# buaacyw/MeshAnything

Hardware: NVIDIA H100
Metric: face-tokens/sec (350M, 800-face cap) (higher is better)
Workload: dtype f16 weights/activations, f32 accumulate

## Files before the change

include/meshanything_b200.h:

```cpp
#ifndef MESHANYTHING_B200_H
#define MESHANYTHING_B200_H

#include <stddef.h>
#include <stdint.h>

#ifdef __cplusplus
extern "C" {
#endif

#define MA_ABI_VERSION 1
#define MA_MAX_LAYERS 32

#define MA_EPI_NONE 0
#define MA_EPI_RELU 1
#define MA_EPI_GELU 2
#define MA_LIN_SEG64 0x10
#define MA_LIN_SEG256 0x20

int ma_abi_version(void);
const char* ma_last_error(void);


int ma_linear_f16(const void* W, const void* bias, const void* x, int ldx, void* y, int ldy, int M, int N, int K,
                  int epilogue, void* stream);

int ma_layernorm(const float* x, const void* res16, const float* gamma, const float* beta, float eps, int M, int W,
                 float* out32, void* out16, void* stream);

size_t ma_attention_scratch_bytes(int M, int H, int max_keys);
int ma_attention_f16(const void* q, int ldq, const void* K, const void* V, long T, int H, const int* slots,
                     const int* nkeys, int max_keys, int M, float scale, void* out, int ldo, void* scratch,
                     void* stream);
int ma_attention_decode_f16(const void* qkv, int ldq, void* K, void* V, long T, const int* nkeys, int max_keys, int M,
                            float scale, void* out, int ldo, void* scratch, void* stream);


typedef struct {
  int n_layers, vocab, codebook, npos;
  const void* wqkv[MA_MAX_LAYERS];
  const void* bqkv[MA_MAX_LAYERS];
  const void* wo[MA_MAX_LAYERS];
  const void* bo[MA_MAX_LAYERS];
  const void* w1[MA_MAX_LAYERS];
  const void* b1[MA_MAX_LAYERS];
  const void* w2[MA_MAX_LAYERS];
  const void* b2[MA_MAX_LAYERS];
  const float* ln1g[MA_MAX_LAYERS];
  const float* ln1b[MA_MAX_LAYERS];
  const float* ln2g[MA_MAX_LAYERS];
  const float* ln2b[MA_MAX_LAYERS];
  const void* lm_head;
  const void* tok_table;
  const float* extra;
  const float* tok_pos;
  const float* cond;
  const float* pos;
} ma_decoder_weights;

typedef struct {
  int do_sample;
  int top_k;
  float top_p;
  uint64_t seed;
} ma_sampling;

int ma_sample_tokens(const void* logits, int B, int vocab, const ma_sampling* sampling, int32_t* out_tokens,
                     int32_t* out_support, void* stream);

size_t ma_kv_cache_bytes(int n_layers, int B, int tmax);
size_t ma_decoder_workspace_bytes(int B, int tmax);

int ma_decode_generate(const ma_decoder_weights* w, const float* prefix, int B, int tmax, int max_new,
                       const ma_sampling* sampling, int eos_id, int pad_id, void* kv, void* ws, int32_t* out_ids,
                       int32_t* out_lens, const int32_t* forced_ids, void* logits_out, int flags, void* stream);

int ma_decode_slots_init(int B, int tmax, int pad_id, void* ws, void* stream);
int ma_decode_slot_stream(int slot, int B, int tmax, int stream_id, void* ws, void* stream);
int ma_decode_slots_seek(int B, int tmax, int pos, int gen, int tok, void* ws, void* stream);
int ma_decode_slot_prefill(const ma_decoder_weights* w, const float* prefix, int slot, int B, int tmax, int max_new,
                           const ma_sampling* sampling, int eos_id, int pad_id, void* kv, void* ws, int32_t* out_ids,
                           void* stream);
int ma_decode_slots_step(const ma_decoder_weights* w, int B, int tmax, int max_new, int n_steps, int max_ctx,
                         const ma_sampling* sampling, int eos_id, int pad_id, void* kv, void* ws, int32_t* out_ids,
                         int flags, void* stream);
int ma_decode_slots_poll(int B, int tmax, void* ws, int32_t* finished_host, int32_t* lens_host, void* stream);

#define MA_GEN_NO_GRAPH 1
#define MA_GEN_NO_FAST 2
#define MA_GEN_NO_PDL 4
#define MA_GEN_NO_EARLY_EXIT 8
#define MA_GEN_NO_MEGA 16
#define MA_GEN_TC 64
#define MA_GEN_TRACE 32

int ma_decoder_debug(void* ws, int B, int tmax, int what, void* host_out, int nbytes);
void ma_mega_set_debug(unsigned long long timeout_ns, int fault);
int ma_decode_persistent_supported(void);


int ma_linear_tc_f16(const void* W, const void* bias, const void* x, int ldx, void* y, int ldy, int M, int N, int K,
                     int epilogue, void* stream);
size_t ma_linear_ws_scratch_bytes(void);
void ma_linear_ws_set_mode(int cluster);
int ma_linear_ws_f16(const void* W, const void* bias, const void* x, int ldx, void* y, int ldy, int M, int N, int K,
                     int epilogue, void* scratch, void* stream);
int ma_set_tensor_cores(int enable);
void ma_tensor_core_linear_counts(unsigned long long* on_tensor_cores, unsigned long long* canonical_fallback);

int ma_attention_tc_f16(const void* q, int ldq, const void* K, const void* Vt, long T, long Tpad, int H,
                        int rows_per_slot, int n_slots, int nkeys, float scale, void* out, int ldo, void* stream);
int ma_transpose_heads_f16(const void* src, int ld, int col0, int head_stride, int H, int n, long Tpad, int n_slots,
                           void* dst, void* stream);


typedef struct {
  const void* c_qkv_w;
  const void *c_proj_w, *c_proj_b;
  const float *ln1_g, *ln1_b, *ln2_g, *ln2_b;
  const void *fc_w, *fc_b;
  const void *proj_w, *proj_b;
} ma_miche_block;

typedef struct {
  const void *input_proj_w, *input_proj_b;
  const float* query;
  const void *cq_w, *ckv_w;
  const void *cproj_w, *cproj_b;
  const float *ln1_g, *ln1_b, *ln2_g, *ln2_b, *ln3_g, *ln3_b;
  const void *fc_w, *fc_b, *proj_w, *proj_b;
  ma_miche_block enc[8];
  const float *lnpost_g, *lnpost_b;
  const void *pre_kl_w, *pre_kl_b;
  const void *post_kl_w, *post_kl_b;
  ma_miche_block dec[16];
  const void *cond_head_w, *cond_head_b;
  const void *cond_w, *cond_b;
} ma_encoder_weights;

size_t ma_encoder_workspace_bytes(int B);

int ma_encoder_forward(const ma_encoder_weights* w, const void* pc_normal, int B, float* point_feature, float* prefix,
                       void* ws, void* stream);


typedef struct {
  const void *in_w, *in_b;
  const void *out_w, *out_b;
  const void *l1_w, *l1_b;
  const void *l2_w, *l2_b;
  const float *n1_g, *n1_b, *n2_g, *n2_b;
} ma_bert_layer;

typedef struct {
  int n_layers;
  ma_bert_layer layer[8];
  const float* pos_embedding;
  const float* point_pe;
  const float *ln_g, *ln_b, *pln_g, *pln_b;
  const void *cond_w, *cond_b, *cond_head_w, *cond_head_b;
  const void *down_w, *down_b;
  const void *coor_w, *coor_b;
  const float* codebook;
} ma_tokenizer_weights;

size_t ma_detokenize_workspace_bytes(int B, int F);

int ma_detokenize(const ma_tokenizer_weights* w, const int32_t* gen_ids, int max_new, int B, int F,
                  const float* point_feature, float* out_xyz, int32_t* ids_out, void* ws, void* stream);

size_t ma_sample_surface_workspace_bytes(int n_faces);
int ma_sample_surface(const float* vertices, const int32_t* faces, int n_faces, int n_samples, unsigned long long seed,
                      void* out_pc_normal, int32_t* out_face_idx, void* ws, void* stream);

unsigned long long ma_launch_count(void);

#ifdef __cplusplus
}
#endif
#endif
```

meshanything_b200/capi.py:

```python
from __future__ import annotations

import ctypes as C
import os
from typing import Optional

import torch

from . import build as _build

MA_MAX_LAYERS = 32
EPI_NONE, EPI_RELU, EPI_GELU = 0, 1, 2
LIN_SEG64, LIN_SEG256 = 0x10, 0x20
GEN_NO_GRAPH, GEN_NO_FAST, GEN_NO_PDL, GEN_NO_EARLY_EXIT, GEN_NO_MEGA, GEN_TRACE, GEN_TC = 1, 2, 4, 8, 16, 32, 64

_vp = C.c_void_p


class DecoderWeights(C.Structure):
    _fields_ = (
        [("n_layers", C.c_int), ("vocab", C.c_int), ("codebook", C.c_int), ("npos", C.c_int)]
        + [(n, _vp * MA_MAX_LAYERS) for n in ("wqkv", "bqkv", "wo", "bo", "w1", "b1", "w2", "b2",
                                              "ln1g", "ln1b", "ln2g", "ln2b")]
        + [(n, _vp) for n in ("lm_head", "tok_table", "extra", "tok_pos", "cond", "pos")]
    )


class Sampling(C.Structure):
    _fields_ = [("do_sample", C.c_int), ("top_k", C.c_int), ("top_p", C.c_float), ("seed", C.c_uint64)]


_lib = None

EXPORTS = [
    "ma_abi_version", "ma_last_error", "ma_launch_count", "ma_linear_f16", "ma_layernorm",
    "ma_attention_scratch_bytes", "ma_attention_f16", "ma_attention_decode_f16", "ma_kv_cache_bytes", "ma_decoder_workspace_bytes",
    "ma_decode_generate", "ma_decoder_debug", "ma_encoder_workspace_bytes", "ma_encoder_forward",
    "ma_detokenize_workspace_bytes", "ma_detokenize", "ma_linear_tc_f16", "ma_set_tensor_cores", "ma_sample_tokens",
    "ma_attention_tc_f16", "ma_transpose_heads_f16",
    "ma_decode_slots_init", "ma_decode_slot_prefill", "ma_decode_slots_step", "ma_decode_slots_poll",
    "ma_mega_set_debug", "ma_linear_ws_set_mode", "ma_decode_slots_seek", "ma_decode_slot_stream", "ma_linear_ws_scratch_bytes", "ma_linear_ws_f16",
    "ma_sample_surface_workspace_bytes", "ma_sample_surface", "ma_tensor_core_linear_counts", "ma_decode_persistent_supported",
]


def lib_path() -> str:
    return _build.LIB


def lib():
    global _lib
    if _lib is not None:
        return _lib
    path = _build.LIB
    dev_tree = os.path.isdir(os.path.join(os.path.dirname(os.path.dirname(os.path.abspath(__file__))), ".git"))
    stale = (os.path.exists(path) and dev_tree and _build.have_nvcc()
             and os.environ.get("MA_B200_NO_AUTOBUILD") != "1" and _build._stale())
    if not os.path.exists(path) or stale or (os.environ.get("MA_B200_REBUILD") == "1"):
        path = _build.build(force=True)
    L = C.CDLL(path)
    L.ma_abi_version.restype = C.c_int
    L.ma_last_error.restype = C.c_char_p
    L.ma_launch_count.restype = C.c_ulonglong
    L.ma_linear_f16.argtypes = [_vp, _vp, _vp, C.c_int, _vp, C.c_int, C.c_int, C.c_int, C.c_int, C.c_int, _vp]
    L.ma_layernorm.argtypes = [_vp, _vp, _vp, _vp, C.c_float, C.c_int, C.c_int, _vp, _vp, _vp]
    L.ma_attention_scratch_bytes.argtypes = [C.c_int, C.c_int, C.c_int]
    L.ma_attention_scratch_bytes.restype = C.c_size_t
    L.ma_attention_f16.argtypes = [_vp, C.c_int, _vp, _vp, C.c_long, C.c_int, _vp, _vp, C.c_int, C.c_int,
                                   C.c_float, _vp, C.c_int, _vp, _vp]
    L.ma_kv_cache_bytes.argtypes = [C.c_int, C.c_int, C.c_int]
    L.ma_kv_cache_bytes.restype = C.c_size_t
    L.ma_decoder_workspace_bytes.argtypes = [C.c_int, C.c_int]
    L.ma_decoder_workspace_bytes.restype = C.c_size_t
    L.ma_decode_generate.argtypes = [C.POINTER(DecoderWeights), _vp, C.c_int, C.c_int, C.c_int, C.POINTER(Sampling),
                                     C.c_int, C.c_int, _vp, _vp, _vp, _vp, _vp, _vp, C.c_int, _vp]
    L.ma_sample_tokens.argtypes = [_vp, C.c_int, C.c_int, C.POINTER(Sampling), _vp, _vp, _vp]
    L.ma_attention_decode_f16.argtypes = [_vp, C.c_int, _vp, _vp, C.c_long, _vp, C.c_int, C.c_int, C.c_float, _vp, C.c_int,
                                          _vp, _vp]
    L.ma_attention_tc_f16.argtypes = [_vp, C.c_int, _vp, _vp, C.c_long, C.c_long, C.c_int, C.c_int, C.c_int, C.c_int,
                                      C.c_float, _vp, C.c_int, _vp]
    L.ma_transpose_heads_f16.argtypes = [_vp, C.c_int, C.c_int, C.c_int, C.c_int, C.c_int, C.c_long, C.c_int, _vp, _vp]
    L.ma_decode_slots_init.argtypes = [C.c_int, C.c_int, C.c_int, _vp, _vp]
    L.ma_linear_ws_set_mode.argtypes = [C.c_int]
    L.ma_linear_ws_set_mode.restype = None
    L.ma_decode_slot_stream.argtypes = [C.c_int, C.c_int, C.c_int, C.c_int, _vp, _vp]
    L.ma_decode_slots_seek.argtypes = [C.c_int, C.c_int, C.c_int, C.c_int, C.c_int, _vp, _vp]
    L.ma_decode_slot_prefill.argtypes = [C.POINTER(DecoderWeights), _vp, C.c_int, C.c_int, C.c_int, C.c_int,
                                         C.POINTER(Sampling), C.c_int, C.c_int, _vp, _vp, _vp, _vp]
    L.ma_decode_slots_step.argtypes = [C.POINTER(DecoderWeights), C.c_int, C.c_int, C.c_int, C.c_int, C.c_int,
                                       C.POINTER(Sampling), C.c_int, C.c_int, _vp, _vp, _vp, C.c_int, _vp]
    L.ma_decode_slots_poll.argtypes = [C.c_int, C.c_int, _vp, _vp, _vp, _vp]
    L.ma_decoder_debug.argtypes = [_vp, C.c_int, C.c_int, C.c_int, _vp, C.c_int]
    L.ma_mega_set_debug.argtypes = [C.c_ulonglong, C.c_int]
    L.ma_mega_set_debug.restype = None
    L.ma_decode_persistent_supported.argtypes = []
    L.ma_decode_persistent_supported.restype = C.c_int
    L.ma_encoder_workspace_bytes.argtypes = [C.c_int]
    L.ma_encoder_workspace_bytes.restype = C.c_size_t
    L.ma_encoder_forward.argtypes = [_vp, _vp, C.c_int, _vp, _vp, _vp, _vp]
    L.ma_detokenize_workspace_bytes.argtypes = [C.c_int, C.c_int]
    L.ma_detokenize_workspace_bytes.restype = C.c_size_t
    L.ma_detokenize.argtypes = [_vp, _vp, C.c_int, C.c_int, C.c_int, _vp, _vp, _vp, _vp, _vp]
    L.ma_linear_ws_scratch_bytes.restype = C.c_size_t
    L.ma_linear_ws_f16.argtypes = [_vp, _vp, _vp, C.c_int, _vp, C.c_int, C.c_int, C.c_int, C.c_int, C.c_int, _vp, _vp]
    L.ma_sample_surface_workspace_bytes.argtypes = [C.c_int]
    L.ma_sample_surface_workspace_bytes.restype = C.c_size_t
    L.ma_sample_surface.argtypes = [_vp, _vp, C.c_int, C.c_int, C.c_ulonglong, _vp, _vp, _vp, _vp]
    L.ma_linear_tc_f16.argtypes = [_vp, _vp, _vp, C.c_int, _vp, C.c_int, C.c_int, C.c_int, C.c_int, C.c_int, _vp]
    L.ma_set_tensor_cores.argtypes = [C.c_int]
    L.ma_tensor_core_linear_counts.argtypes = [C.POINTER(C.c_ulonglong), C.POINTER(C.c_ulonglong)]
    L.ma_tensor_core_linear_counts.restype = None
    if L.ma_abi_version() != 1:
        raise RuntimeError("libmeshanything_b200.so: ABI version mismatch")
    _lib = L
    return L


def check(rc: int, what: str):
    if rc != 0:
        raise RuntimeError(f"{what} failed: {lib().ma_last_error().decode()}")


def ptr(t: Optional[torch.Tensor]):
    return None if t is None else C.c_void_p(t.data_ptr())


def stream_ptr() -> C.c_void_p:
    return C.c_void_p(torch.cuda.current_stream().cuda_stream)


def _need_cuda(*ts):
    for t in ts:
        if t is not None and not t.is_cuda:
            raise RuntimeError("meshanything_b200: tensors must live on a CUDA device (no CPU fallback)")



def linear_f16(w: torch.Tensor, bias: Optional[torch.Tensor], x: torch.Tensor, epilogue: int = EPI_NONE,
               out: Optional[torch.Tensor] = None) -> torch.Tensor:
    _need_cuda(w, bias, x)
    assert w.dtype == torch.float16 and x.dtype == torch.float16 and w.is_contiguous()
    assert x.dim() == 2 and x.stride(1) == 1
    M, K = x.shape
    N = w.shape[0]
    if out is None:
        out = torch.empty((M, N), dtype=torch.float16, device=x.device)
    check(lib().ma_linear_f16(ptr(w), ptr(bias), ptr(x), x.stride(0), ptr(out), out.stride(0), M, N, K, epilogue,
                              stream_ptr()), "ma_linear_f16")
    return out


def sample_surface(vertices: torch.Tensor, faces: torch.Tensor, n_samples: int, seed: int = 0,
                   want_index: bool = False):
    _need_cuda(vertices, faces)
    v = vertices.to(torch.float32).contiguous()
    f = faces.to(torch.int32).contiguous()
    F = f.shape[0]
    ws = torch.empty(lib().ma_sample_surface_workspace_bytes(F), dtype=torch.uint8, device=v.device)
    out = torch.empty((n_samples, 6), dtype=torch.float16, device=v.device)
    idx = torch.empty((n_samples,), dtype=torch.int32, device=v.device) if want_index else None
    check(lib().ma_sample_surface(ptr(v), ptr(f), F, n_samples, int(seed), ptr(out), ptr(idx), ptr(ws), stream_ptr()),
          "ma_sample_surface")
    return (out, idx) if want_index else out


def tensor_core_linear_counts():
    a, b = C.c_ulonglong(0), C.c_ulonglong(0)
    lib().ma_tensor_core_linear_counts(C.byref(a), C.byref(b))
    return a.value, b.value


_ws_scratch = {}


def linear_ws_f16(w: torch.Tensor, bias: Optional[torch.Tensor], x: torch.Tensor, epilogue: int = EPI_NONE) -> torch.Tensor:
    _need_cuda(w, bias, x)
    M, K = x.shape
    N = w.shape[0]
    scr = _ws_scratch.get(x.device)
    if scr is None:
        scr = _ws_scratch[x.device] = torch.zeros(lib().ma_linear_ws_scratch_bytes(), dtype=torch.uint8, device=x.device)
    out = torch.empty((M, N), dtype=torch.float16, device=x.device)
    check(lib().ma_linear_ws_f16(ptr(w), ptr(bias), ptr(x), x.stride(0), ptr(out), out.stride(0), M, N, K, epilogue,
                                 ptr(scr), stream_ptr()), "ma_linear_ws_f16")
    return out


def linear_tc_f16(w: torch.Tensor, bias: Optional[torch.Tensor], x: torch.Tensor, epilogue: int = EPI_NONE) -> torch.Tensor:
    _need_cuda(w, bias, x)
    M, K = x.shape
    N = w.shape[0]
    out = torch.empty((M, N), dtype=torch.float16, device=x.device)
    check(lib().ma_linear_tc_f16(ptr(w), ptr(bias), ptr(x), x.stride(0), ptr(out), out.stride(0), M, N, K, epilogue,
                                 stream_ptr()), "ma_linear_tc_f16")
    return out


def transpose_heads_f16(src: torch.Tensor, col0: int, head_stride: int, H: int, n: int, n_slots: int) -> torch.Tensor:
    _need_cuda(src)
    Tpad = (n + 127) // 128 * 128
    dst = torch.empty((n_slots, H, 64, Tpad), dtype=torch.float16, device=src.device)
    check(lib().ma_transpose_heads_f16(ptr(src), src.stride(0), col0, head_stride, H, n, Tpad, n_slots, ptr(dst),
                                       stream_ptr()), "ma_transpose_heads_f16")
    return dst


def attention_tc_f16(q: torch.Tensor, k: torch.Tensor, vt: torch.Tensor, nkeys: int, rows_per_slot: int,
                     scale: float = 0.125) -> torch.Tensor:
    _need_cuda(q, k, vt)
    S, H, T, _ = k.shape
    Tpad = vt.shape[3]
    assert q.is_contiguous() and k.is_contiguous() and vt.is_contiguous() and q.shape[0] == S * rows_per_slot
    out = torch.empty_like(q)
    check(lib().ma_attention_tc_f16(ptr(q), q.stride(0), ptr(k), ptr(vt), T, Tpad, H, rows_per_slot, S, nkeys,
                                    C.c_float(scale), ptr(out), out.stride(0), stream_ptr()), "ma_attention_tc_f16")
    return out


def sample_tokens(logits: torch.Tensor, do_sample: bool = True, top_k: int = 50, top_p: float = 0.95, seed: int = 0,
                  want_support: bool = False):
    _need_cuda(logits)
    assert logits.dtype == torch.float16 and logits.is_contiguous()
    B, vocab = logits.shape
    tok = torch.empty((B,), dtype=torch.int32, device=logits.device)
    sup = torch.empty((B, 256), dtype=torch.int32, device=logits.device) if want_support else None
    s = Sampling(int(do_sample), int(top_k), float(top_p), int(seed))
    check(lib().ma_sample_tokens(ptr(logits), B, vocab, C.byref(s), ptr(tok), ptr(sup), stream_ptr()),
          "ma_sample_tokens")
    return (tok, sup) if want_support else tok


def layernorm(x: Optional[torch.Tensor], res16: Optional[torch.Tensor], gamma: torch.Tensor, beta: torch.Tensor,
              eps: float = 1e-5, want32: bool = True, want16: bool = True):
    _need_cuda(x, res16, gamma, beta)
    src = x if x is not None else res16
    M, W = src.shape
    o32 = torch.empty((M, W), dtype=torch.float32, device=src.device) if want32 else None
    o16 = torch.empty((M, W), dtype=torch.float16, device=src.device) if want16 else None
    check(lib().ma_layernorm(ptr(x), ptr(res16), ptr(gamma), ptr(beta), eps, M, W, ptr(o32), ptr(o16), stream_ptr()),
          "ma_layernorm")
    return o32, o16


def attention_decode_f16(qkv: torch.Tensor, k: torch.Tensor, v: torch.Tensor, nkeys: torch.Tensor,
                         scale: float = 0.125) -> torch.Tensor:
    _need_cuda(qkv, k, v, nkeys)
    M = qkv.shape[0]
    assert qkv.shape[1] == 3072 and qkv.is_contiguous() and k.is_contiguous() and v.is_contiguous()
    assert k.shape[0] == M and k.shape[1] == 16 and k.shape[3] == 64
    T = k.shape[2]
    max_keys = int(nkeys.max().item())
    scratch = torch.zeros(lib().ma_attention_scratch_bytes(M, 16, max_keys), dtype=torch.uint8, device=qkv.device)
    out = torch.empty((M, 1024), dtype=torch.float16, device=qkv.device)
    check(lib().ma_attention_decode_f16(ptr(qkv), 3072, ptr(k), ptr(v), T, ptr(nkeys), max_keys, M, scale, ptr(out),
                                        1024, ptr(scratch), stream_ptr()), "ma_attention_decode_f16")
    return out


def attention_f16(q: torch.Tensor, k: torch.Tensor, v: torch.Tensor, nkeys: torch.Tensor,
                  slots: Optional[torch.Tensor] = None, scale: float = 0.125) -> torch.Tensor:
    _need_cuda(q, k, v, nkeys, slots)
    M, H, D = q.shape
    assert D == 64 and k.is_contiguous() and v.is_contiguous() and q.is_contiguous()
    T = k.shape[2]
    max_keys = int(nkeys.max().item())
    scratch = torch.zeros(lib().ma_attention_scratch_bytes(M, H, max_keys), dtype=torch.uint8, device=q.device)
    out = torch.empty((M, H, D), dtype=torch.float16, device=q.device)
    check(lib().ma_attention_f16(ptr(q), H * D, ptr(k), ptr(v), T, H, ptr(slots), ptr(nkeys), max_keys, M, scale,
                                 ptr(out), H * D, ptr(scratch), stream_ptr()), "ma_attention_f16")
    return out
```

meshanything_b200/csrc/api.cu:

```cuda
#include <stdarg.h>
#include <stdlib.h>
#include <stdio.h>
#include <string.h>

#include <atomic>
#include <map>
#include <mutex>
#include <vector>

#include "canon.cuh"
#include "internal.h"

namespace ma {

static thread_local char g_err[512] = "";
static std::atomic<unsigned long long> g_launches{0};

void set_error(const char* fmt, ...) {
  va_list ap;
  va_start(ap, fmt);
  vsnprintf(g_err, sizeof(g_err), fmt, ap);
  va_end(ap);
}
void count_launch(int n) { g_launches += (unsigned long long)n; }
bool check_launch(const char* what) {
  cudaError_t e = cudaPeekAtLastError();
  if (e != cudaSuccess) {
    set_error("%s: %s", what, cudaGetErrorString(e));
    cudaGetLastError();
    return false;
  }
  return true;
}

static inline size_t align_up(size_t x, size_t a = 256) { return (x + a - 1) / a * a; }

constexpr int PREFILL_SEQS = 8;

struct DecWs {
  float* hres;
  __half *x16, *qkv, *attn16, *y16, *f16, *logits, *lastx16;
  int* nkeys;
  SeqState s;
  int* all_done;
  void* attn_scratch;
  size_t attn_scratch_bytes;
  void* attn_scratch_pre;
  size_t attn_scratch_pre_bytes;
  void* fast;
  void* mega;
  void* tc_scratch;
  size_t total;
};

static DecWs carve(void* base, int B, int tmax, int vocab) {
  DecWs w;
  const size_t rows = (size_t)std::max(B, PREFIX * std::min(B, PREFILL_SEQS));
  size_t off = 0;
  auto take = [&](size_t bytes) {
    void* p = base ? (void*)((char*)base + off) : nullptr;
    off += align_up(bytes);
    return p;
  };
  w.hres = (float*)take(rows * HID * 4);
  w.x16 = (__half*)take(rows * HID * 2);
  w.qkv = (__half*)take(rows * QKV * 2);
  w.attn16 = (__half*)take(rows * HID * 2);
  w.y16 = (__half*)take(rows * HID * 2);
  w.f16 = (__half*)take(rows * FFN * 2);
  w.logits = (__half*)take((size_t)B * vocab * 2);
  w.lastx16 = (__half*)take((size_t)B * HID * 2);
  w.nkeys = (int*)take(rows * 4);
  w.s.pos = (int*)take((size_t)B * 4);
  w.s.gen = (int*)take((size_t)B * 4);
  w.s.tok = (int*)take((size_t)B * 4);
  w.s.finished = (int*)take((size_t)B * 4);
  w.s.lens = (int*)take((size_t)B * 4);
  w.s.sid = (int*)take((size_t)B * 4);
  w.all_done = (int*)take(256);
  w.attn_scratch_bytes = attention_scratch_bytes((int)B, NHEAD, tmax);
  w.attn_scratch = take(w.attn_scratch_bytes);
  w.attn_scratch_pre_bytes = attention_scratch_bytes(PREFIX * std::min(B, PREFILL_SEQS), NHEAD, PREFIX);
  w.attn_scratch_pre = take(w.attn_scratch_pre_bytes);
  w.fast = take(fast_workspace_bytes());
  w.mega = take(mega_workspace_bytes());
  w.tc_scratch = take(linear_ws_scratch_bytes());
  w.total = off;
  return w;
}

static inline __half* kv_layer(void* kv, int layer, int which, int B, long T) {
  return (__half*)kv + ((size_t)(layer * 2 + which) * B) * NHEAD * T * HD;
}

static const bool g_no_stream_attn = [] {
  const char* e = getenv("MA_B200_NO_STREAM_ATTN");
  return e && e[0] == '1';
}();

static const bool g_no_pdl = [] {
  const char* e = getenv("MA_B200_NO_PDL");
  return e && e[0] == '1';
}();

static int dec_linear(bool tc, const DecWs& ws, const void* W, const void* b, const __half* x, int ldx, __half* y, int ldy,
                      int M, int N, int K, int epi, cudaStream_t st, bool pdl = false) {
  if (tc) {
    const bool tiled_ok = M >= 64 && linear_tc_supported(M, N, K, ldx, ldy, x, W, y);
    const bool ws_ok = M <= 128 && linear_ws_supported(M, N, K, ldx, x, W);
    if (ws_ok && (linear_ws_mode() || !tiled_ok || K > 1024))
      return launch_linear_ws((const __half*)W, (const __half*)b, x, ldx, y, ldy, M, N, K, epi, ws.tc_scratch, st, pdl);
    if (tiled_ok) return launch_linear_tc((const __half*)W, (const __half*)b, x, ldx, y, ldy, M, N, K, epi, st);
  }
  return launch_linear((const __half*)W, (const __half*)b, x, ldx, y, ldy, M, N, K, epi, st);
}

static int run_layers(const ma_decoder_weights* w, const DecWs& ws, void* kv, int B, long T, int M, int rows_per_slot,
                      int slot0, int max_keys, cudaStream_t st, bool tc = false) {
  void* scratch = rows_per_slot > 1 ? ws.attn_scratch_pre : ws.attn_scratch;
  const bool pdl = tc && rows_per_slot == 1 && !g_no_pdl;
  for (int L = 0; L < w->n_layers; L++) {
    __half* kc = kv_layer(kv, L, 0, B, T) + (size_t)slot0 * NHEAD * T * HD;
    __half* vc = kv_layer(kv, L, 1, B, T) + (size_t)slot0 * NHEAD * T * HD;
    if (dec_linear(tc, ws, w->wqkv[L], w->bqkv[L], ws.x16, HID, ws.qkv, QKV, M, QKV, HID, MA_EPI_NONE, st, pdl)) return 1;
    if (rows_per_slot == 1 && !g_no_stream_attn) {
      if (launch_attention_decode(ws.qkv, QKV, kc, vc, T, ws.nkeys, max_keys, M, 0.125f, ws.attn16, HID, scratch, pdl,
                                  st)) return 1;
    } else {
      if (launch_kv_append(ws.qkv, M, rows_per_slot, ws.nkeys, kc, vc, T, st)) return 1;
      if (launch_attention(ws.qkv, QKV, kc, vc, T, NHEAD, rows_per_slot, nullptr, ws.nkeys, max_keys, M, 0.125f,
                           ws.attn16, HID, scratch, st)) return 1;
    }
    if (dec_linear(tc, ws, w->wo[L], w->bo[L], ws.attn16, HID, ws.y16, HID, M, HID, HID, MA_EPI_NONE, st, pdl)) return 1;
    if (launch_layernorm(ws.hres, ws.y16, w->ln1g[L], w->ln1b[L], MA_LN_EPS, M, HID, ws.hres, ws.x16, st, pdl)) return 1;
    if (dec_linear(tc, ws, w->w1[L], w->b1[L], ws.x16, HID, ws.f16, FFN, M, FFN, HID, MA_EPI_RELU, st, pdl)) return 1;
    if (dec_linear(tc, ws, w->w2[L], w->b2[L], ws.f16, FFN, ws.y16, HID, M, HID, FFN, MA_EPI_NONE, st, pdl)) return 1;
    if (launch_layernorm(ws.hres, ws.y16, w->ln2g[L], w->ln2b[L], MA_LN_EPS, M, HID, ws.hres, ws.x16, st, pdl)) return 1;
  }
  return 0;
}

struct GraphKey {
  const void *w, *kv, *ws, *out_ids, *forced, *logits_out;
  unsigned long long whash;
  int B, tmax, max_new, bucket, flags, do_sample, top_k, eos, pad, mode;
  float top_p;
  unsigned long long seed;
  bool operator<(const GraphKey& o) const { return memcmp(this, &o, sizeof(GraphKey)) < 0; }
};
static std::map<GraphKey, cudaGraphExec_t> g_graphs;
static std::map<cudaGraphExec_t, unsigned long long> g_graph_launches;
static cudaStream_t g_stream = nullptr;
static int* g_flag_host = nullptr;
static cudaEvent_t g_ev_in = nullptr, g_ev_out = nullptr, g_ev_flag = nullptr;

static int g_device = -1;
static std::mutex g_mu;

static int ensure_globals() {
  int dev = -1;
  if (cudaGetDevice(&dev) != cudaSuccess) {
    set_error("cudaGetDevice: %s", cudaGetErrorString(cudaGetLastError()));
    return 1;
  }
  if (g_device >= 0 && dev != g_device) {
    set_error("ma_decode_generate was first used on device %d; this process now runs on device %d "
              "(one process per GPU)", g_device, dev);
    return 1;
  }
  if (!g_stream) {
    if (cudaStreamCreateWithFlags(&g_stream, cudaStreamNonBlocking) != cudaSuccess ||
        cudaHostAlloc((void**)&g_flag_host, 64, cudaHostAllocDefault) != cudaSuccess ||
        cudaEventCreateWithFlags(&g_ev_in, cudaEventDisableTiming) != cudaSuccess ||
        cudaEventCreateWithFlags(&g_ev_out, cudaEventDisableTiming) != cudaSuccess ||
        cudaEventCreateWithFlags(&g_ev_flag, cudaEventDisableTiming) != cudaSuccess) {
      set_error("cannot create stream/events: %s", cudaGetErrorString(cudaGetLastError()));
      return 1;
    }
    g_device = dev;
  }
  return 0;
}


static int enqueue_batched_step(const ma_decoder_weights* w, const DecWs& ws, void* kv, int B, long T, int max_keys,
                                const SampleArgs& sa, cudaStream_t s, bool tc) {
  if (launch_embed_tokens(w, ws.s, B, ws.hres, ws.x16, ws.nkeys, s)) return 1;
  if (run_layers(w, ws, kv, B, T, B, 1, 0, max_keys, s, tc)) return 1;
  if (dec_linear(tc, ws, w->lm_head, nullptr, ws.x16, HID, ws.logits, w->vocab, B, w->vocab, HID, MA_EPI_NONE, s,
                 tc && !g_no_pdl)) return 1;
  return launch_sample(sa, s);
}

static inline bool use_tc(int B, int do_sample, int flags) { return B > 1 && (do_sample || (flags & MA_GEN_TC)); }

static unsigned long long weights_hash(const ma_decoder_weights* w) {
  unsigned long long h = 1469598103934665603ull;
  const unsigned char* pb = (const unsigned char*)w;
  for (size_t q = 0; q < sizeof(ma_decoder_weights); q++) h = (h ^ pb[q]) * 1099511628211ull;
  return h;
}

template <class F>
static int launch_cached_graph(const GraphKey& key, cudaStream_t st, F&& enqueue) {
  auto it = g_graphs.find(key);
  if (it == g_graphs.end()) {
    cudaGraph_t graph = nullptr;
    if (cudaStreamBeginCapture(st, cudaStreamCaptureModeThreadLocal) != cudaSuccess) {
      set_error("cudaStreamBeginCapture: %s", cudaGetErrorString(cudaGetLastError()));
      return 1;
    }
    const unsigned long long before = g_launches.load();
    int erc = enqueue(st);
    const unsigned long long per_step = g_launches.load() - before;
    cudaError_t ce = cudaStreamEndCapture(st, &graph);
    if (erc || ce != cudaSuccess || !graph) {
      if (!erc) set_error("cudaStreamEndCapture: %s", cudaGetErrorString(ce));
      cudaGetLastError();
      return 1;
    }
    cudaGraphExec_t exec = nullptr;
    ce = cudaGraphInstantiate(&exec, graph, 0);
    cudaGraphDestroy(graph);
    if (ce != cudaSuccess) {
      set_error("cudaGraphInstantiate: %s", cudaGetErrorString(ce));
      return 1;
    }
    if (g_graphs.size() > 64) {
      for (auto& kvp : g_graphs) cudaGraphExecDestroy(kvp.second);
      g_graphs.clear();
      g_graph_launches.clear();
    }
    it = g_graphs.emplace(key, exec).first;
    g_launches -= per_step;
    g_graph_launches[exec] = per_step;
  }
  if (cudaGraphLaunch(it->second, st) != cudaSuccess) {
    set_error("cudaGraphLaunch: %s", cudaGetErrorString(cudaGetLastError()));
    return 1;
  }
  g_launches += g_graph_launches[it->second];
  return 0;
}

static void fill_sample_args(SampleArgs& sa, const ma_decoder_weights* w, const DecWs& ws, int B, int max_new,
                             const ma_sampling* sampling, int eos_id, int pad_id, int32_t* out_ids) {
  memset(&sa, 0, sizeof(sa));
  sa.logits = ws.logits; sa.vocab = w->vocab; sa.B = B; sa.max_new = max_new; sa.eos_id = eos_id; sa.pad_id = pad_id;
  sa.do_sample = sampling ? sampling->do_sample : 0;
  sa.top_k = sampling ? sampling->top_k : 0;
  sa.top_p = sampling ? sampling->top_p : 1.0f;
  sa.seed = sampling ? sampling->seed : 0;
  sa.s = ws.s; sa.out_ids = out_ids;
}

static int check_decode_args(const char* who, const ma_decoder_weights* w, int B, int tmax, int max_new) {
  if (w->n_layers > MA_MAX_LAYERS || w->vocab > 8195 + 61) {
    set_error("%s: n_layers=%d / vocab=%d unsupported", who, w->n_layers, w->vocab);
    return 1;
  }
  if (B <= 0 || max_new <= 0 || PREFIX + max_new > tmax) {
    set_error("%s: B=%d, tmax=%d < 257 + max_new=%d", who, B, tmax, max_new);
    return 1;
  }
  if (PREFIX + max_new + 2 > w->npos) {
    set_error("%s: sequence of %d exceeds %d learned positions", who, PREFIX + max_new, w->npos - 2);
    return 1;
  }
  return 0;
}

}

using namespace ma;

extern "C" {

int ma_abi_version(void) { return MA_ABI_VERSION; }
const char* ma_last_error(void) { return g_err; }
unsigned long long ma_launch_count(void) { return g_launches.load(); }

int ma_linear_f16(const void* W, const void* bias, const void* x, int ldx, void* y, int ldy, int M, int N, int K,
                  int epilogue, void* stream) {
  return launch_linear((const __half*)W, (const __half*)bias, (const __half*)x, ldx, (__half*)y, ldy, M, N, K,
                       epilogue, (cudaStream_t)stream);
}

size_t ma_linear_ws_scratch_bytes(void) { return linear_ws_scratch_bytes(); }
void ma_linear_ws_set_mode(int cluster) { linear_ws_set_mode(cluster); }

int ma_linear_ws_f16(const void* W, const void* bias, const void* x, int ldx, void* y, int ldy, int M, int N, int K,
                     int epilogue, void* scratch, void* stream) {
  return launch_linear_ws((const __half*)W, (const __half*)bias, (const __half*)x, ldx, (__half*)y, ldy, M, N, K,
                          epilogue, scratch, (cudaStream_t)stream);
}

int ma_layernorm(const float* x, const void* res16, const float* gamma, const float* beta, float eps, int M, int W,
                 float* out32, void* out16, void* stream) {
  return launch_layernorm(x, (const __half*)res16, gamma, beta, eps, M, W, out32, (__half*)out16,
                          (cudaStream_t)stream);
}

size_t ma_attention_scratch_bytes(int M, int H, int max_keys) { return attention_scratch_bytes(M, H, max_keys); }

int ma_attention_f16(const void* q, int ldq, const void* K, const void* V, long T, int H, const int* slots,
                     const int* nkeys, int max_keys, int M, float scale, void* out, int ldo, void* scratch,
                     void* stream) {
  if (M > 65535) {
    set_error("ma_attention_f16: M=%d exceeds 65535 rows per call", M);
    return 1;
  }
  return launch_attention((const __half*)q, ldq, (const __half*)K, (const __half*)V, T, H, 1, slots, nkeys, max_keys, M,
                          scale, (__half*)out, ldo, scratch, (cudaStream_t)stream);
}

int ma_attention_decode_f16(const void* qkv, int ldq, void* K, void* V, long T, const int* nkeys, int max_keys, int M,
                            float scale, void* out, int ldo, void* scratch, void* stream) {
  if (!qkv || !K || !V || !nkeys || !out || !scratch || M < 1 || max_keys < 1 || max_keys > T || ldq < 3 * HID) {
    set_error("ma_attention_decode_f16: bad arguments (M=%d, max_keys=%d, T=%ld, ldq=%d)", M, max_keys, T, ldq);
    return 1;
  }
  return launch_attention_decode((const __half*)qkv, ldq, (__half*)K, (__half*)V, T, nkeys, max_keys, M, scale,
                                 (__half*)out, ldo, scratch, false, (cudaStream_t)stream);
}

int ma_sample_tokens(const void* logits, int B, int vocab, const ma_sampling* sampling, int32_t* out_tokens,
                     int32_t* out_support, void* stream) {
  if (!logits || !out_tokens || B < 1 || vocab < 1) {
    set_error("ma_sample_tokens: bad arguments");
    return 1;
  }
  SampleArgs sa;
  memset(&sa, 0, sizeof(sa));
  sa.logits = (const __half*)logits; sa.vocab = vocab; sa.B = B; sa.max_new = 1; sa.eos_id = -1; sa.pad_id = -1;
  sa.do_sample = sampling ? sampling->do_sample : 0;
  sa.top_k = sampling ? sampling->top_k : 0;
  sa.top_p = sampling ? sampling->top_p : 1.0f;
  sa.seed = sampling ? sampling->seed : 0;
  sa.first = 1; sa.token_out = out_tokens; sa.support_out = out_support;
  return launch_sample(sa, (cudaStream_t)stream);
}

size_t ma_kv_cache_bytes(int n_layers, int B, int tmax) {
  return (size_t)n_layers * 2 * B * NHEAD * (size_t)tmax * HD * sizeof(__half);
}

size_t ma_decoder_workspace_bytes(int B, int tmax) { return carve(nullptr, B, tmax, 8195 + 61).total; }

int ma_decode_generate(const ma_decoder_weights* w, const float* prefix, int B, int tmax, int max_new,
                       const ma_sampling* sampling, int eos_id, int pad_id, void* kv, void* ws_, int32_t* out_ids,
                       int32_t* out_lens, const int32_t* forced_ids, void* logits_out, int flags, void* stream) {
  if (!w || !prefix || !kv || !ws_ || !out_ids || B <= 0 || max_new <= 0) {
    set_error("ma_decode_generate: bad arguments");
    return 1;
  }
  if (check_decode_args("ma_decode_generate", w, B, tmax, max_new)) return 1;
  std::lock_guard<std::mutex> lock(g_mu);
  if (ensure_globals()) return 1;
  cudaStream_t user = (cudaStream_t)stream;
  cudaStream_t st = g_stream;
  cudaEventRecord(g_ev_in, user);
  cudaStreamWaitEvent(st, g_ev_in, 0);

  const long T = tmax;
  DecWs ws = carve(ws_, B, tmax, 8195 + 61);
  cudaMemsetAsync(ws.attn_scratch, 0, ws.attn_scratch_bytes, st);
  cudaMemsetAsync(ws.attn_scratch_pre, 0, ws.attn_scratch_pre_bytes, st);
  cudaMemsetAsync(ws.fast, 0, fast_workspace_bytes(), st);
  if (launch_fill_i32(out_ids, pad_id, (long)B * max_new, st)) return 1;

  SampleArgs sa;
  fill_sample_args(sa, w, ws, B, max_new, sampling, eos_id, pad_id, out_ids);
  sa.first = 1; sa.forced = forced_ids; sa.logits_out = (__half*)logits_out;
  sa.all_done = ws.all_done;

  const bool tc = use_tc(B, sa.do_sample, flags);
  if (tc) cudaMemsetAsync(ws.tc_scratch, 0, linear_ws_scratch_bytes(), st);
  const bool fast = (B == 1) && !(flags & MA_GEN_NO_FAST);
  bool mega = fast && !sa.do_sample && !(flags & MA_GEN_NO_MEGA) && mega_fits(tmax) && mega_supported();
  if (fast) sa.nkeys_next = fast_nkeys_ptr(ws.fast);
  if (mega && mega_prepare(w, ws.mega, st)) mega = false;

  for (int b0 = 0; b0 < B; b0 += PREFILL_SEQS) {
    const int nb = std::min(PREFILL_SEQS, B - b0), M = nb * PREFIX;
    if (launch_embed_prefix(w, prefix + (size_t)b0 * PREFIX * HID, nb, ws.hres, ws.x16, ws.nkeys, st)) return 1;
    if (run_layers(w, ws, kv, B, T, M, PREFIX, b0, PREFIX, st, tc)) return 1;
    if (launch_gather_rows(ws.x16, HID, PREFIX - 1, PREFIX, nb, ws.lastx16 + (size_t)b0 * HID, st)) return 1;
  }
  if (dec_linear(tc, ws, w->lm_head, nullptr, ws.lastx16, HID, ws.logits, w->vocab, B, w->vocab, HID, MA_EPI_NONE, st))
    return 1;
  if (launch_sample(sa, st)) return 1;
  sa.first = 0;
  sa.nkeys_next = nullptr;


  const bool use_graph = !(flags & MA_GEN_NO_GRAPH);
  const bool early = !(flags & MA_GEN_NO_EARLY_EXIT) && !forced_ids;
  const int CHECK_EVERY = 64;
  const unsigned long long whash = use_graph ? weights_hash(w) : 0;
  bool flag_pending = false;
  int rc = 0;
  if (mega) {
    const int MEGA_STEPS = 512;
    for (int i = 1; i < max_new && rc == 0; i += MEGA_STEPS) {
      rc = mega_enqueue(w, ws.s, tmax, (__half*)kv, ws.mega, sa, std::min(MEGA_STEPS, max_new - i), i - 1,
                        (flags & MA_GEN_TRACE) ? 1 : 0, st);
    }
  }
  for (int i = 1; i < max_new && rc == 0 && !mega; i++) {
    const int ctx = PREFIX + i;
    const int bucket = fast ? 0 : (ctx + 1023) / 1024;
    const int max_keys = fast ? tmax : std::min(tmax, bucket * 1024);
    auto enqueue = [&](cudaStream_t s) -> int {
      if (fast) return fast_step_enqueue(w, ws.s, tmax, (__half*)kv, ws.fast, sa, !(flags & MA_GEN_NO_PDL), s);
      return enqueue_batched_step(w, ws, kv, B, T, max_keys, sa, s, tc);
    };
    if (!use_graph) {
      rc = enqueue(st);
    } else {
      GraphKey key;
      memset(&key, 0, sizeof(key));
      key.w = w; key.kv = kv; key.ws = ws_; key.out_ids = out_ids; key.forced = forced_ids; key.logits_out = logits_out;
      key.B = B; key.tmax = tmax; key.max_new = max_new; key.bucket = bucket; key.flags = flags;
      key.do_sample = sa.do_sample; key.top_k = sa.top_k; key.eos = eos_id; key.pad = pad_id; key.top_p = sa.top_p;
      key.seed = sa.do_sample ? sa.seed : 0;
      key.whash = whash;
      if (launch_cached_graph(key, st, enqueue)) return 1;
    }
    if (early && (i % CHECK_EVERY) == 0) {
      if (flag_pending && cudaEventQuery(g_ev_flag) == cudaSuccess) {
        if (*g_flag_host == 1) break;
        flag_pending = false;
      }
      if (!flag_pending) {
        cudaMemcpyAsync(g_flag_host, ws.all_done, sizeof(int), cudaMemcpyDeviceToHost, st);
        cudaEventRecord(g_ev_flag, st);
        flag_pending = true;
      }
    }
  }
  if (rc) return rc;
  if (out_lens) cudaMemcpyAsync(out_lens, ws.s.lens, sizeof(int) * B, cudaMemcpyDeviceToDevice, st);
  cudaEventRecord(g_ev_out, st);
  cudaStreamWaitEvent(user, g_ev_out, 0);
  return check_launch("ma_decode_generate") ? 0 : 1;
}



static int slots_enter(void* stream, cudaStream_t* st) {
  if (ensure_globals()) return 1;
  cudaEventRecord(g_ev_in, (cudaStream_t)stream);
  cudaStreamWaitEvent(g_stream, g_ev_in, 0);
  *st = g_stream;
  return 0;
}
static int slots_leave(void* stream, const char* who) {
  cudaEventRecord(g_ev_out, g_stream);
  cudaStreamWaitEvent((cudaStream_t)stream, g_ev_out, 0);
  return check_launch(who) ? 0 : 1;
}

int ma_decode_slots_init(int B, int tmax, int pad_id, void* ws_, void* stream) {
  if (!ws_ || B <= 0 || tmax < PREFIX + 1) {
    set_error("ma_decode_slots_init: bad arguments");
    return 1;
  }
  std::lock_guard<std::mutex> lock(g_mu);
  cudaStream_t st;
  if (slots_enter(stream, &st)) return 1;
  DecWs ws = carve(ws_, B, tmax, 8195 + 61);
  cudaMemsetAsync(ws.attn_scratch, 0, ws.attn_scratch_bytes, st);
  cudaMemsetAsync(ws.attn_scratch_pre, 0, ws.attn_scratch_pre_bytes, st);
  cudaMemsetAsync(ws.tc_scratch, 0, linear_ws_scratch_bytes(), st);
  if (launch_fill_i32(ws.s.pos, PREFIX, B, st) || launch_fill_i32(ws.s.gen, 0, B, st) ||
      launch_fill_i32(ws.s.tok, pad_id, B, st) || launch_fill_i32(ws.s.finished, 1, B, st) ||
      launch_fill_i32(ws.s.lens, 0, B, st) || launch_fill_i32(ws.s.sid, 0, B, st)) return 1;
  return slots_leave(stream, "ma_decode_slots_init");
}

int ma_decode_slot_stream(int slot, int B, int tmax, int stream_id, void* ws_, void* stream) {
  if (!ws_ || slot < 0 || slot >= B) {
    set_error("ma_decode_slot_stream: bad arguments (slot %d of %d)", slot, B);
    return 1;
  }
  std::lock_guard<std::mutex> lock(g_mu);
  cudaStream_t st;
  if (slots_enter(stream, &st)) return 1;
  DecWs ws = carve(ws_, B, tmax, 8195 + 61);
  if (launch_fill_i32(ws.s.sid + slot, stream_id, 1, st)) return 1;
  return slots_leave(stream, "ma_decode_slot_stream");
}

int ma_decode_slots_seek(int B, int tmax, int pos, int gen, int tok, void* ws_, void* stream) {
  if (!ws_ || B <= 0 || pos < PREFIX || pos >= tmax || gen < 1) {
    set_error("ma_decode_slots_seek: bad arguments (pos %d of tmax %d)", pos, tmax);
    return 1;
  }
  std::lock_guard<std::mutex> lock(g_mu);
  cudaStream_t st;
  if (slots_enter(stream, &st)) return 1;
  DecWs ws = carve(ws_, B, tmax, 8195 + 61);
  if (launch_fill_i32(ws.s.pos, pos, B, st) || launch_fill_i32(ws.s.gen, gen, B, st) ||
      launch_fill_i32(ws.s.tok, tok, B, st) || launch_fill_i32(ws.s.finished, 0, B, st) ||
      launch_fill_i32(ws.s.lens, gen, B, st)) return 1;
  return slots_leave(stream, "ma_decode_slots_seek");
}

int ma_decode_slot_prefill(const ma_decoder_weights* w, const float* prefix, int slot, int B, int tmax, int max_new,
                           const ma_sampling* sampling, int eos_id, int pad_id, void* kv, void* ws_, int32_t* out_ids,
                           void* stream) {
  if (!w || !prefix || !kv || !ws_ || !out_ids || slot < 0 || slot >= B) {
    set_error("ma_decode_slot_prefill: bad arguments (slot %d of %d)", slot, B);
    return 1;
  }
  if (check_decode_args("ma_decode_slot_prefill", w, B, tmax, max_new)) return 1;
  std::lock_guard<std::mutex> lock(g_mu);
  cudaStream_t st;
  if (slots_enter(stream, &st)) return 1;
  const long T = tmax;
  DecWs ws = carve(ws_, B, tmax, 8195 + 61);
  if (launch_fill_i32(out_ids + (size_t)slot * max_new, pad_id, max_new, st)) return 1;
  if (launch_embed_prefix(w, prefix, 1, ws.hres, ws.x16, ws.nkeys, st)) return 1;
  const bool tc = use_tc(B, sampling ? sampling->do_sample : 0, 0);
  if (run_layers(w, ws, kv, B, T, PREFIX, PREFIX, slot, PREFIX, st, tc)) return 1;
  __half* last = ws.lastx16 + (size_t)slot * HID;
  if (launch_gather_rows(ws.x16, HID, PREFIX - 1, PREFIX, 1, last, st)) return 1;
  if (dec_linear(tc, ws, w->lm_head, nullptr, last, HID, ws.logits + (size_t)slot * w->vocab, w->vocab, 1, w->vocab, HID,
                 MA_EPI_NONE, st)) return 1;
  SampleArgs sa;
  fill_sample_args(sa, w, ws, B, max_new, sampling, eos_id, pad_id, out_ids);
  sa.first = 1; sa.row0 = slot; sa.nrows = 1; sa.slots = 1;
  if (launch_sample(sa, st)) return 1;
  return slots_leave(stream, "ma_decode_slot_prefill");
}

int ma_decode_slots_step(const ma_decoder_weights* w, int B, int tmax, int max_new, int n_steps, int max_ctx,
                         const ma_sampling* sampling, int eos_id, int pad_id, void* kv, void* ws_, int32_t* out_ids,
                         int flags, void* stream) {
  if (!w || !kv || !ws_ || !out_ids || n_steps < 0 || max_ctx < PREFIX + 1) {
    set_error("ma_decode_slots_step: bad arguments");
    return 1;
  }
  if (check_decode_args("ma_decode_slots_step", w, B, tmax, max_new)) return 1;
  std::lock_guard<std::mutex> lock(g_mu);
  cudaStream_t st;
  if (slots_enter(stream, &st)) return 1;
  const long T = tmax;
  DecWs ws = carve(ws_, B, tmax, 8195 + 61);
  SampleArgs sa;
  fill_sample_args(sa, w, ws, B, max_new, sampling, eos_id, pad_id, out_ids);
  sa.slots = 1;
  const bool use_graph = !(flags & MA_GEN_NO_GRAPH);
  const unsigned long long whash = use_graph ? weights_hash(w) : 0;
  for (int i = 0; i < n_steps; i++) {
    const int ctx = std::min(tmax, max_ctx + i);
    const int bucket = (ctx + 1023) / 1024;
    const int max_keys = std::min(tmax, bucket * 1024);
    auto enqueue = [&](cudaStream_t s) -> int {
      return enqueue_batched_step(w, ws, kv, B, T, max_keys, sa, s, use_tc(B, sa.do_sample, flags));
    };
    if (!use_graph) {
      if (enqueue(st)) return 1;
    } else {
      GraphKey key;
      memset(&key, 0, sizeof(key));
      key.w = w; key.kv = kv; key.ws = ws_; key.out_ids = out_ids;
      key.B = B; key.tmax = tmax; key.max_new = max_new; key.bucket = bucket; key.flags = flags; key.mode = 1;
      key.do_sample = sa.do_sample; key.top_k = sa.top_k; key.eos = eos_id; key.pad = pad_id; key.top_p = sa.top_p;
      key.seed = sa.do_sample ? sa.seed : 0;
      if (launch_cached_graph(key, st, enqueue)) return 1;
    }
  }
  return slots_leave(stream, "ma_decode_slots_step");
}

int ma_decode_slots_poll(int B, int tmax, void* ws_, int32_t* finished_host, int32_t* lens_host, void* stream) {
  if (!ws_ || !finished_host || !lens_host || B <= 0) {
    set_error("ma_decode_slots_poll: bad arguments");
    return 1;
  }
  std::lock_guard<std::mutex> lock(g_mu);
  cudaStream_t st;
  if (slots_enter(stream, &st)) return 1;
  DecWs ws = carve(ws_, B, tmax, 8195 + 61);
  cudaMemcpyAsync(finished_host, ws.s.finished, sizeof(int) * B, cudaMemcpyDeviceToHost, st);
  cudaMemcpyAsync(lens_host, ws.s.lens, sizeof(int) * B, cudaMemcpyDeviceToHost, st);
  if (cudaStreamSynchronize(st) != cudaSuccess) {
    set_error("ma_decode_slots_poll: %s", cudaGetErrorString(cudaGetLastError()));
    return 1;
  }
  return slots_leave(stream, "ma_decode_slots_poll");
}


void ma_mega_set_debug(unsigned long long timeout_ns, int fault) { mega_set_debug(timeout_ns, fault); }
int ma_decode_persistent_supported(void) { return mega_supported(); }

int ma_decoder_debug(void* ws_, int B, int tmax, int what, void* host_out, int nbytes) {
  DecWs ws = carve(ws_, B, tmax, 8195 + 61);
  cudaDeviceSynchronize();
  if (what == 0 && !mega_supported()) {
    memset(host_out, 0, (size_t)nbytes);
    return 0;
  }
  const char* src = (const char*)ws.mega + (what == 0 ? mega_error_flag_offset() : what == 1 ? mega_trace_offset() : mega_trace_cta_offset());
  return cudaMemcpy(host_out, src, (size_t)nbytes, cudaMemcpyDeviceToHost) == cudaSuccess ? 0 : 1;
}

}
```

meshanything_b200/csrc/decode_mega.cu:

```cuda
#include "canon.cuh"
#include "internal.h"

namespace ma {

constexpr int MG_THREADS = 512;
constexpr int MG_WARPS = 16;
constexpr int TEAM = 256;
constexpr int PARTF = 66;
constexpr int MAX_CHUNKS = 72;

struct MegaWs {
  uint2 qkv_w[QKV / 2];
  uint2 attn_w[HID / 2];
  uint2 ya_w[HID / 2];
  uint2 yb_w[HID / 2];
  uint2 f_w[FFN / 2];
  uint2 cand_w[256 * 2];
  int error;
  int pad_[3];
  unsigned long long trace[1280];
  unsigned long long trace_cta[160 * 8];
  ma_decoder_weights w;
  alignas(256) uint2 part_w[NHEAD * MAX_CHUNKS * PARTF];
  alignas(256) __half bias_cta[MA_MAX_LAYERS * 160 * 128];
};

constexpr int BIAS_QKV = 0, BIAS_OUT = 32, BIAS_FC1 = 48, BIAS_FC2 = 112;

struct MegaArgs {
  MegaWs* ws;
  SeqState s;
  __half* kv;
  long T;
  int n_steps, step_base, max_new, eos_id, pad_id;
  int rows_qkv, rows_out, rows_fc1, rows_fc2, rows_lm;
  int32_t* out_ids;
  const int32_t* forced;
  __half* logits_out;
  int* all_done;
  int* nkeys_next;
  int trace;
  int fault;
};

__device__ __forceinline__ unsigned long long gtimer() {
  unsigned long long t;
  asm volatile("mov.u64 %0, %globaltimer;" : "=l"(t));
  return t;
}

__device__ __forceinline__ void ll_store(uint2* p, uint32_t data, uint32_t ep) {
  asm volatile("st.volatile.global.v2.u32 [%0], {%1,%2};" ::"l"(p), "r"(data), "r"(ep) : "memory");
}
__device__ __forceinline__ uint4 ll_load2(const uint2* p) {
  uint4 v;
  asm volatile("ld.volatile.global.v4.u32 {%0,%1,%2,%3}, [%4];" : "=r"(v.x), "=r"(v.y), "=r"(v.z), "=r"(v.w) : "l"(p) : "memory");
  return v;
}
__device__ __forceinline__ uint2 ll_load1(const uint2* p) {
  uint2 v;
  asm volatile("ld.volatile.global.v2.u32 {%0,%1}, [%2];" : "=r"(v.x), "=r"(v.y) : "l"(p) : "memory");
  return v;
}
__constant__ unsigned c_spin_limit = 1u << 24;
#define SPIN_LIMIT c_spin_limit
__device__ __forceinline__ bool poll_giveup(int* err, unsigned& spins) {
  if ((++spins & 1023u) == 0) {
    if (*reinterpret_cast<volatile int*>(err)) return true;
    if (spins > SPIN_LIMIT) {
      atomicCAS(err, 0, 1 + (int)blockIdx.x);
      return true;
    }
  }
  return false;
}
__device__ __forceinline__ uint2 ll_wait2(const uint2* p, uint32_t ep, int* err) {
  uint4 v = ll_load2(p);
  unsigned spins = 0;
  while (v.y != ep || v.w != ep) {
    if (poll_giveup(err, spins)) break;
    v = ll_load2(p);
  }
  return make_uint2(v.x, v.z);
}
__device__ __forceinline__ uint32_t ll_wait1(const uint2* p, uint32_t ep, int* err) {
  uint2 v = ll_load1(p);
  unsigned spins = 0;
  while (v.y != ep) {
    if (poll_giveup(err, spins)) break;
    v = ll_load1(p);
  }
  return v.x;
}
template <int N>
__device__ __forceinline__ void ll_wait_units(const uint2* p, int stride, uint32_t ep, uint2* out, int* err) {
  uint4 v[N];
#pragma unroll
  for (int i = 0; i < N; i++) v[i] = ll_load2(p + 2 * i * stride);
  unsigned spins = 0;
  for (;;) {
    bool ok = true;
#pragma unroll
    for (int i = 0; i < N; i++) {
      if (v[i].y != ep || v[i].w != ep) {
        ok = false;
        v[i] = ll_load2(p + 2 * i * stride);
      }
    }
    if (ok) break;
    if (poll_giveup(err, spins)) break;
  }
#pragma unroll
  for (int i = 0; i < N; i++) out[i] = make_uint2(v[i].x, v[i].z);
}
__device__ __forceinline__ void store_x4(float* dst, uint2 d) {
  const __half2* hh = reinterpret_cast<const __half2*>(&d);
  const float2 p0 = __half22float2(hh[0]), p1 = __half22float2(hh[1]);
  *reinterpret_cast<float4*>(dst) = make_float4(p0.x, p0.y, p1.x, p1.y);
}
__device__ __forceinline__ void ll_gather(const uint2* src, int nhalf, uint32_t ep, __half* dst, int* err) {
  const int tid = threadIdx.x;
  if (nhalf == FFN) {
    uint2 d[2];
    ll_wait_units<2>(src + 2 * tid, MG_THREADS, ep, d, err);
    *reinterpret_cast<uint2*>(dst + 4 * tid) = d[0];
    *reinterpret_cast<uint2*>(dst + 4 * (tid + MG_THREADS)) = d[1];
  } else {
    for (int u = tid; u < nhalf / 4; u += MG_THREADS) {
      const uint2 d = ll_wait2(src + 2 * u, ep, err);
      *reinterpret_cast<uint2*>(dst + 4 * u) = d;
    }
  }
}

struct alignas(128) MegaSmem {
  uint64_t bar[4];
  uint64_t lnbar[2];
  uint64_t bbar[2];
  alignas(16) float ln1[2 * HID];
  alignas(16) float ln2[2 * HID];
  alignas(16) __half bias[2][128];
  ma_decoder_weights wtab;
  int errflag;
  float red[2][8];
  float wmax[2][8];
  float ared[2][8][65];
  float bval[MG_WARPS];
  int bidx[MG_WARPS];
  float cstage[2 * 2 * MAX_CHUNKS];
  alignas(16) __half stage16[64];
  alignas(16) float hres[HID];
  alignas(16) __half xs[FFN];
};

__device__ __forceinline__ uint4 ldcg16(const void* p) { return __ldcg(reinterpret_cast<const uint4*>(p)); }
__device__ __forceinline__ void fence_proxy_async() { asm volatile("fence.proxy.async.shared::cta;" ::: "memory"); }

__device__ __forceinline__ void layernorm_1024(float* v, const float* gamma, const float* beta, float (*red)[8], int tid) {
  if (tid >= 256) return;
  const int warp = tid >> 5, lane = tid & 31;
  const float inv = __fdiv_rn(1.0f, 1024.0f);
  float p = fadd(fadd(v[0], v[1]), fadd(v[2], v[3]));
  p = warp_sum(p);
  if (lane == 0) red[0][warp] = p;
  asm volatile("bar.sync 3, 256;" ::: "memory");
  const float mean = fmul(warp_tree(red[0], 8), inv);
  const float d0 = fsub(v[0], mean), d1 = fsub(v[1], mean), d2 = fsub(v[2], mean), d3 = fsub(v[3], mean);
  float q = fadd(fadd(fmul(d0, d0), fmul(d1, d1)), fadd(fmul(d2, d2), fmul(d3, d3)));
  q = warp_sum(q);
  if (lane == 0) red[1][warp] = q;
  asm volatile("bar.sync 3, 256;" ::: "memory");
  const float var = fmul(warp_tree(red[1], 8), inv);
  const float rstd = __fdiv_rn(1.0f, __fsqrt_rn(fadd(var, MA_LN_EPS)));
  const float4 g = *reinterpret_cast<const float4*>(gamma + 4 * tid);
  const float4 b = *reinterpret_cast<const float4*>(beta + 4 * tid);
  v[0] = ffma(fmul(d0, rstd), g.x, b.x);
  v[1] = ffma(fmul(d1, rstd), g.y, b.y);
  v[2] = ffma(fmul(d2, rstd), g.z, b.z);
  v[3] = ffma(fmul(d3, rstd), g.w, b.w);
}

__device__ __forceinline__ void team_sync(int team) { asm volatile("bar.sync %0, %1;" ::"r"(1 + team), "r"(TEAM) : "memory"); }

__device__ __forceinline__ void load_x8(const float* p, float* xf) {
  const float4 a = *reinterpret_cast<const float4*>(p), b = *reinterpret_cast<const float4*>(p + 4);
  xf[0] = a.x; xf[1] = a.y; xf[2] = a.z; xf[3] = a.w; xf[4] = b.x; xf[5] = b.y; xf[6] = b.z; xf[7] = b.w;
}

template <int K, bool RELU>
__device__ __forceinline__ void gemv_stage(const __half* sw, int nrows, const __half* bias, const __half* xs, int warp,
                                           int lane, __half* stage) {
  constexpr int G = K / 256;
  if (warp >= nrows) return;
  const __half* w[4];
  bool has[4];
#pragma unroll
  for (int i = 0; i < 4; i++) {
    const int r = warp + MG_WARPS * i;
    has[i] = r < nrows;
    w[i] = sw + (size_t)(has[i] ? r : warp) * K + 8 * lane;
  }
  float acc[4] = {0.0f, 0.0f, 0.0f, 0.0f};
  if (!has[1]) {
#pragma unroll 4
    for (int g = 0; g < G; g++) {
      float xf[8], f[8];
      unpack8(*reinterpret_cast<const uint4*>(xs + 256 * g + 8 * lane), xf);
      unpack8(*reinterpret_cast<const uint4*>(w[0] + 256 * g), f);
#pragma unroll
      for (int j = 0; j < 8; j++) acc[0] = ffma(f[j], xf[j], acc[0]);
    }
  } else if (!has[2]) {
#pragma unroll 4
    for (int g = 0; g < G; g++) {
      float xf[8], f0[8], f1[8];
      unpack8(*reinterpret_cast<const uint4*>(xs + 256 * g + 8 * lane), xf);
      unpack8(*reinterpret_cast<const uint4*>(w[0] + 256 * g), f0);
      unpack8(*reinterpret_cast<const uint4*>(w[1] + 256 * g), f1);
#pragma unroll
      for (int j = 0; j < 8; j++) {
        acc[0] = ffma(f0[j], xf[j], acc[0]);
        acc[1] = ffma(f1[j], xf[j], acc[1]);
      }
    }
  } else {
#pragma unroll 2
    for (int g = 0; g < G; g++) {
      float xf[8], f[4][8];
      unpack8(*reinterpret_cast<const uint4*>(xs + 256 * g + 8 * lane), xf);
#pragma unroll
      for (int i = 0; i < 4; i++) unpack8(*reinterpret_cast<const uint4*>(w[i] + 256 * g), f[i]);
#pragma unroll
      for (int j = 0; j < 8; j++) {
#pragma unroll
        for (int i = 0; i < 4; i++) acc[i] = ffma(f[i][j], xf[j], acc[i]);
      }
    }
  }
#pragma unroll
  for (int i = 0; i < 4; i++) {
    if (i == 0 || has[1]) acc[i] = warp_sum(acc[i]);
  }
  if (lane == 0) {
#pragma unroll
    for (int i = 0; i < 4; i++) {
      if (has[i]) {
        const int r = warp + MG_WARPS * i;
        __half h = __float2half_rn(fadd(acc[i], bias ? __half2float(bias[r]) : 0.0f));
        if (RELU && __half2float(h) < 0.0f) h = __float2half_rn(0.0f);
        stage[r] = h;
      }
    }
  }
}

__device__ __forceinline__ uint32_t pack2(__half a, __half b) {
  return (uint32_t)__half_as_ushort(a) | ((uint32_t)__half_as_ushort(b) << 16);
}

__device__ __forceinline__ void refill(__half* dst, const void* W, int row0, int nrows, int K, uint64_t* bar) {
  fence_proxy_async();
  if (nrows > 0) {
    const uint32_t bytes = (uint32_t)nrows * K * 2;
    mbar_expect_tx(bar, bytes);
    bulk_g2s(dst, reinterpret_cast<const __half*>(W) + (size_t)row0 * K, bytes, bar);
  } else {
    mbar_expect_tx(bar, 0);
  }
}

__device__ __forceinline__ void fill_ln(float* dst, const float* g, const float* b, uint64_t* bar) {
  fence_proxy_async();
  mbar_expect_tx(bar, 2u * HID * 4);
  bulk_g2s(dst, g, HID * 4, bar);
  bulk_g2s(dst + HID, b, HID * 4, bar);
}
__device__ __forceinline__ void fill_bias(__half* dst, const __half* src, uint64_t* bar) {
  fence_proxy_async();
  mbar_expect_tx(bar, 256);
  bulk_g2s(dst, src, 256, bar);
}

__global__ void __launch_bounds__(MG_THREADS, 1) decode_mega_kernel(MegaArgs a) {
  extern __shared__ __align__(128) unsigned char smem_raw[];
  MegaSmem& sm = *reinterpret_cast<MegaSmem*>(smem_raw);
  __half* bufD = reinterpret_cast<__half*>(smem_raw + sizeof(MegaSmem));
  __half* bufC = bufD + (size_t)a.rows_qkv * HID;
  __half* bufA = bufC + (size_t)a.rows_out * HID;
  __half* bufB = bufA + (size_t)a.rows_fc1 * HID;
  const int tid = threadIdx.x, warp = tid >> 5, lane = tid & 31;
  const int team = warp >> 3, wt = warp & 7, tl = tid & (TEAM - 1);
  const int grp = lane >> 3, li = lane & 7;
  MegaWs* ws = a.ws;
  {
    const uint32_t* src = reinterpret_cast<const uint32_t*>(&ws->w);
    uint32_t* dst = reinterpret_cast<uint32_t*>(&sm.wtab);
    for (int i = tid; i < (int)(sizeof(ma_decoder_weights) / 4); i += MG_THREADS) dst[i] = src[i];
  }
  if (tid == 0) sm.errflag = *reinterpret_cast<volatile int*>(&ws->error);
  __syncthreads();
  if (sm.errflag) return;
  const ma_decoder_weights& W = sm.wtab;
  const int NL = W.n_layers;
  const long T = a.T;
  int* err = &ws->error;

  const int cta = blockIdx.x, ncta = gridDim.x;
  const int row0_qkv = cta * a.rows_qkv, n_qkv = max(0, min(a.rows_qkv, QKV - row0_qkv));
  const int row0_out = cta * a.rows_out, n_out = max(0, min(a.rows_out, HID - row0_out));
  const int row0_fc1 = cta * a.rows_fc1, n_fc1 = max(0, min(a.rows_fc1, FFN - row0_fc1));
  const int row0_fc2 = cta * a.rows_fc2, n_fc2 = max(0, min(a.rows_fc2, HID - row0_fc2));
  const int row0_lm = cta * a.rows_lm, n_lm = max(0, min(a.rows_lm, W.vocab - row0_lm));
  const int lmD = min(n_lm, a.rows_qkv), lmC = max(0, min(n_lm, a.rows_qkv + a.rows_out) - a.rows_qkv),
            lmA = max(0, n_lm - a.rows_qkv - a.rows_out);

  uint32_t parD = 0, parC = 0, parA = 0, parB = 0, parL1 = 0, parL2 = 0, parB0 = 0, parB1 = 0;
  int lc = 0;
  if (tid == 0) {
    for (int i = 0; i < 4; i++) mbar_init(&sm.bar[i], 1);
    for (int i = 0; i < 2; i++) { mbar_init(&sm.lnbar[i], 1); mbar_init(&sm.bbar[i], 1); }
    mbar_fence_init();
    fill_ln(sm.ln1, W.ln1g[0], W.ln1b[0], &sm.lnbar[0]);
    fill_ln(sm.ln2, W.ln2g[0], W.ln2b[0], &sm.lnbar[1]);
    fill_bias(sm.bias[0], ws->bias_cta + ((size_t)0 * 160 + cta) * 128, &sm.bbar[0]);
    fill_bias(sm.bias[1], ws->bias_cta + ((size_t)(NL > 1 ? 1 : 0) * 160 + cta) * 128, &sm.bbar[1]);
    refill(bufD, W.wqkv[0], row0_qkv, n_qkv, HID, &sm.bar[0]);
    refill(bufC, W.wo[0], row0_out, n_out, HID, &sm.bar[1]);
    refill(bufA, W.w1[0], row0_fc1, n_fc1, HID, &sm.bar[2]);
    refill(bufB, W.w2[0], row0_fc2, n_fc2, FFN, &sm.bar[3]);
  }
  __syncthreads();

  int pos = a.s.pos[0], gen = a.s.gen[0], tok = a.s.tok[0], fin = a.s.finished[0];
  unsigned long long* tr = (a.trace && cta == 0 && tid == 0) ? ws->trace : nullptr;
  int tri = 0;
#define STAMP() do { if (tr && tri < 1270) tr[tri++] = gtimer(); } while (0)
#define CSTAMP(k) do { if (a.trace && tid == 0 && step == 1 && L == NL / 2) ws->trace_cta[cta * 8 + (k)] = gtimer(); } while (0)

  auto publish_x = [&](const float* v, bool keep_hres) {
    if (tid < 256) {
      if (keep_hres) *reinterpret_cast<float4*>(sm.hres + 4 * tid) = make_float4(v[0], v[1], v[2], v[3]);
      __half2 h0 = __floats2half2_rn(v[0], v[1]), h1 = __floats2half2_rn(v[2], v[3]);
      uint2 u;
      u.x = *reinterpret_cast<uint32_t*>(&h0);
      u.y = *reinterpret_cast<uint32_t*>(&h1);
      *reinterpret_cast<uint2*>(sm.xs + 4 * tid) = u;
    }
  };
  auto residual_in = [&](const uint2* words, uint32_t ep, float* v) {
    if (tid < 256) {
      const float4 hv = *reinterpret_cast<const float4*>(sm.hres + 4 * tid);
      const uint2 d = ll_wait2(words + 2 * tid, ep, err);
      const __half2* hh = reinterpret_cast<const __half2*>(&d);
      const float2 p0 = __half22float2(hh[0]), p1 = __half22float2(hh[1]);
      v[0] = fadd(hv.x, p0.x); v[1] = fadd(hv.y, p0.y); v[2] = fadd(hv.z, p1.x); v[3] = fadd(hv.w, p1.y);
    } else {
      v[0] = v[1] = v[2] = v[3] = 0.0f;
    }
  };

  for (int step = 0; step < a.n_steps; step++) {
    if (gen >= a.max_new || fin) break;
    const int nkeys = pos + 1;
    const int nch = (nkeys + MA_ATTN_CHUNK - 1) / MA_ATTN_CHUNK;
    const int nitems = nch * NHEAD;
    const uint32_t ep0 = (uint32_t)(a.step_base + step) * (uint32_t)NL + 1u;
    STAMP();

    for (int L = 0; L < NL; L++) {
      const uint32_t ep = ep0 + (uint32_t)L;
      const int bsel = lc & 1;
      const __half* lb = sm.bias[bsel];
      __half* kc = a.kv + ((size_t)(L * 2 + 0)) * NHEAD * T * HD;
      __half* vc = a.kv + ((size_t)(L * 2 + 1)) * NHEAD * T * HD;

      uint4 kreg[8], vreg[8];
      int item = team * ncta + (ncta - 1 - cta);
      if (item < nitems) {
        const int c = item >> 4, h = item & 15;
        const long base = ((long)h * T + (long)c * MA_ATTN_CHUNK) * HD;
#pragma unroll
        for (int rho = 0; rho < 8; rho++) {
          const int r = 32 * rho + 4 * wt + grp;
          if (c * MA_ATTN_CHUNK + r < pos) {
            kreg[rho] = ldcg16(kc + base + (long)r * HD + 8 * li);
            vreg[rho] = ldcg16(vc + base + (long)r * HD + 8 * li);
          }
        }
      }

      {
        float v[4] = {0.0f, 0.0f, 0.0f, 0.0f};
        if (L == 0) {
          if (tid < 256) {
            float4 X;
            int fidx;
            if (tok < 3) {
              X = *reinterpret_cast<const float4*>(W.extra + (long)tok * HID + 4 * tid);
              fidx = tok;
            } else {
              const uint2 u = *reinterpret_cast<const uint2*>(reinterpret_cast<const __half*>(W.tok_table) +
                                                              (long)(tok - 3) * HID + 4 * tid);
              const __half2* hh = reinterpret_cast<const __half2*>(&u);
              const float2 p0 = __half22float2(hh[0]), p1 = __half22float2(hh[1]);
              X = make_float4(p0.x, p0.y, p1.x, p1.y);
              int r = (gen - 2) % 9;
              if (r < 0) r += 9;
              fidx = r + 3;
            }
            const float4 F = *reinterpret_cast<const float4*>(W.tok_pos + (long)fidx * HID + 4 * tid);
            const float4 C = *reinterpret_cast<const float4*>(W.cond + HID + 4 * tid);
            const float4 P = *reinterpret_cast<const float4*>(W.pos + (long)(pos + 2) * HID + 4 * tid);
            v[0] = fadd(fadd(fadd(X.x, F.x), C.x), P.x);
            v[1] = fadd(fadd(fadd(X.y, F.y), C.y), P.y);
            v[2] = fadd(fadd(fadd(X.z, F.z), C.z), P.z);
            v[3] = fadd(fadd(fadd(X.w, F.w), C.w), P.w);
          }
        } else {
          residual_in(ws->yb_w, ep - 1, v);
          mbar_wait(&sm.lnbar[1], parL2);
          parL2 ^= 1;
          layernorm_1024(v, sm.ln2, sm.ln2 + HID, sm.red, tid);
        }
        publish_x(v, true);
      }
      __syncthreads();
      if (L > 0 && tid == 0) fill_ln(sm.ln2, W.ln2g[L], W.ln2b[L], &sm.lnbar[1]);
      STAMP();
      CSTAMP(0);
      mbar_wait(&sm.bbar[bsel], bsel ? parB1 : parB0);
      if (bsel) parB1 ^= 1; else parB0 ^= 1;
      mbar_wait(&sm.bar[0], parD);
      parD ^= 1;
      STAMP();
      gemv_stage<HID, false>(bufD, n_qkv, lb + BIAS_QKV, sm.xs, warp, lane, sm.stage16);
      STAMP();
      __syncthreads();
      STAMP();
      if (tid < (n_qkv >> 1)) {
        const int n = row0_qkv + 2 * tid;
        const uint32_t d = *reinterpret_cast<const uint32_t*>(sm.stage16 + 2 * tid);
        ll_store(ws->qkv_w + (n >> 1), d, ep);
        if (n >= HID) {
          const int e = (n - HID) & (HID - 1), head = e >> 6, dd = e & 63;
          __half* c = (n < 2 * HID) ? kc : vc;
          *reinterpret_cast<uint32_t*>(c + ((long)head * T + pos) * HD + dd) = d;
        }
      }
      if (tid == 0) {
        if (L + 1 < NL) refill(bufD, W.wqkv[L + 1], row0_qkv, n_qkv, HID, &sm.bar[0]);
        else refill(bufD, W.lm_head, row0_lm, lmD, HID, &sm.bar[0]);
      }
      STAMP();
      CSTAMP(1);

      for (int it = 0; item < nitems; item += 2 * ncta, it++) {
        const int c = item >> 4, h = item & 15;
        const int len = min(MA_ATTN_CHUNK, nkeys - c * MA_ATTN_CHUNK);
        const long base = ((long)h * T + (long)c * MA_ATTN_CHUNK) * HD;
        const int cur = pos - c * MA_ATTN_CHUNK;
#pragma unroll
        for (int rho = 0; rho < 8; rho++) {
          const int r = 32 * rho + 4 * wt + grp;
          if (r < len && it > 0 && r != cur) {
            kreg[rho] = ldcg16(kc + base + (long)r * HD + 8 * li);
            vreg[rho] = ldcg16(vc + base + (long)r * HD + 8 * li);
          }
        }
        float qf[8];
        {
          uint2 d[2];
          ll_wait_units<2>(ws->qkv_w + (h * HD + 8 * li) / 2, 1, ep, d, err);
          unpack8(make_uint4(d[0].x, d[0].y, d[1].x, d[1].y), qf);
        }
        if (cur >= 0 && cur < MA_ATTN_CHUNK) {
          const int rho_c = cur >> 5, gl_c = cur & 31;
          if (4 * wt + grp == gl_c) {
            uint2 kk[2], vv[2];
            ll_wait_units<2>(ws->qkv_w + (HID + h * HD + 8 * li) / 2, 1, ep, kk, err);
            ll_wait_units<2>(ws->qkv_w + (2 * HID + h * HD + 8 * li) / 2, 1, ep, vv, err);
            const uint2 k0 = kk[0], k1 = kk[1], v0 = vv[0], v1 = vv[1];
#pragma unroll
            for (int rho = 0; rho < 8; rho++)
              if (rho == rho_c) {
                kreg[rho] = make_uint4(k0.x, k0.y, k1.x, k1.y);
                vreg[rho] = make_uint4(v0.x, v0.y, v1.x, v1.y);
              }
          }
        }
        float pr[8];
#pragma unroll
        for (int rho = 0; rho < 8; rho++) {
          float kf[8];
          unpack8(kreg[rho], kf);
          float p = 0.0f;
#pragma unroll
          for (int j = 0; j < 8; j++) p = ffma(qf[j], kf[j], p);
          pr[rho] = p;
        }
#pragma unroll
        for (int sft = 4; sft >= 1; sft >>= 1) {
          const bool up = (li & sft) != 0;
#pragma unroll
          for (int i = 0; i < sft; i++) {
            const float mine = up ? pr[i + sft] : pr[i];
            const float other = up ? pr[i] : pr[i + sft];
            pr[i] = fadd(mine, __shfl_xor_sync(0xffffffffu, other, sft));
          }
        }
        const float s_own = fmul(pr[0], 0.125f);
        const bool own_valid = 32 * li + 4 * wt + grp < len;
        float lmax = own_valid ? s_own : -INFINITY;
        lmax = warp_max(lmax);
        team_sync(team);
        if (lane == 0) sm.wmax[team][wt] = lmax;
        team_sync(team);
        float cmax = sm.wmax[team][0];
#pragma unroll
        for (int w2 = 1; w2 < 8; w2++) cmax = fmaxf(cmax, sm.wmax[team][w2]);
        const float e_own = own_valid ? ma_exp(fsub(s_own, cmax)) : 0.0f;
        float l = 0.0f, o[8];
#pragma unroll
        for (int j = 0; j < 8; j++) o[j] = 0.0f;
#pragma unroll
        for (int rho = 0; rho < 8; rho++) {
          const int r = 32 * rho + 4 * wt + grp;
          const float e = __shfl_sync(0xffffffffu, e_own, (lane & 24) | rho);
          if (r < len) {
            l = fadd(l, e);
            const float pf = __half2float(__float2half_rn(e));
            float vf[8];
            unpack8(vreg[rho], vf);
#pragma unroll
            for (int j = 0; j < 8; j++) o[j] = ffma(pf, vf[j], o[j]);
          }
        }
        l = fadd(l, __shfl_xor_sync(0xffffffffu, l, 16));
        l = fadd(l, __shfl_xor_sync(0xffffffffu, l, 8));
#pragma unroll
        for (int j = 0; j < 8; j++) {
          o[j] = fadd(o[j], __shfl_xor_sync(0xffffffffu, o[j], 16));
          o[j] = fadd(o[j], __shfl_xor_sync(0xffffffffu, o[j], 8));
        }
        if (grp == 0) {
#pragma unroll
          for (int j = 0; j < 8; j++) sm.ared[team][wt][8 * li + j] = o[j];
          if (li == 0) sm.ared[team][wt][64] = l;
        }
        team_sync(team);
        if (tl < 65) {
          float x[8];
#pragma unroll
          for (int w2 = 0; w2 < 8; w2++) x[w2] = sm.ared[team][w2][tl];
          const float rsum = fadd(fadd(fadd(x[0], x[1]), fadd(x[2], x[3])), fadd(fadd(x[4], x[5]), fadd(x[6], x[7])));
          uint2* part = ws->part_w + ((long)h * MAX_CHUNKS + c) * PARTF;
          ll_store(part + (tl < 64 ? tl : 65), __float_as_uint(rsum), ep);
          if (tl == 64) ll_store(part + 64, __float_as_uint(cmax), ep);
        }
      }
      if (tl == 0) {
        const int Ln = (L + 1 < NL) ? L + 1 : 0;
        const __half* kn = a.kv + ((size_t)(Ln * 2 + 0)) * NHEAD * T * HD;
        const __half* vn = a.kv + ((size_t)(Ln * 2 + 1)) * NHEAD * T * HD;
        for (int it2 = team * ncta + (ncta - 1 - cta); it2 < nitems; it2 += 2 * ncta) {
          const int c2 = it2 >> 4, h2 = it2 & 15;
          const uint32_t bytes = (uint32_t)min(MA_ATTN_CHUNK, nkeys - c2 * MA_ATTN_CHUNK) * HD * 2;
          const long off = ((long)h2 * T + (long)c2 * MA_ATTN_CHUNK) * HD;
          asm volatile("cp.async.bulk.prefetch.L2.global [%0], %1;" ::"l"(kn + off), "r"(bytes) : "memory");
          asm volatile("cp.async.bulk.prefetch.L2.global [%0], %1;" ::"l"(vn + off), "r"(bytes) : "memory");
        }
      }
      STAMP();
      CSTAMP(2);
      if (team == 0 && ncta - 1 - cta < NHEAD) {
        const int h = ncta - 1 - cta;
        const uint2* part = ws->part_w + (long)h * MAX_CHUNKS * PARTF;
        float* ost = reinterpret_cast<float*>(sm.xs);
        float* wgt = sm.cstage + team * 2 * MAX_CHUNKS;
        float* mst = wgt + MAX_CHUNKS;
        const bool single = nch <= 31;
        team_sync(team);
        if (!single) {
          for (int i = tl; i < nch; i += TEAM) mst[i] = __uint_as_float(ll_wait1(part + (long)i * PARTF + 64, ep, err));
          team_sync(team);
          float M = -INFINITY;
          for (int cc = 0; cc < nch; cc++) M = fmaxf(M, mst[cc]);
          for (int i = tl; i < nch; i += TEAM) wgt[i] = ma_exp(fsub(mst[i], M));
        }
        float Lsum = 0.0f, O = 0.0f;
        for (int c0 = 0; c0 < nch; c0 += 31) {
          const int nb = min(31, nch - c0), nw = nb * PARTF;
          {
            uint2 w[8];
#pragma unroll
            for (int k = 0; k < 8; k++) {
              const int i = tl + TEAM * k;
              if (i < nw) w[k] = ll_load1(part + (long)c0 * PARTF + i);
            }
            unsigned spins = 0;
            for (;;) {
              bool ok = true;
#pragma unroll
              for (int k = 0; k < 8; k++) {
                const int i = tl + TEAM * k;
                if (i < nw && w[k].y != ep) {
                  ok = false;
                  w[k] = ll_load1(part + (long)c0 * PARTF + i);
                }
              }
              if (ok) break;
              if (poll_giveup(err, spins)) break;
            }
#pragma unroll
            for (int k = 0; k < 8; k++) {
              const int i = tl + TEAM * k;
              if (i < nw) ost[i] = __uint_as_float(w[k].x);
            }
          }
          team_sync(team);
          if (single) {
            float M = -INFINITY;
            for (int cc = 0; cc < nch; cc++) M = fmaxf(M, ost[cc * PARTF + 64]);
            for (int i = tl; i < nch; i += TEAM) wgt[i] = ma_exp(fsub(ost[i * PARTF + 64], M));
            team_sync(team);
          }
          if (tl < 64) {
            for (int cc = 0; cc < nb; cc++) {
              const float wc = wgt[c0 + cc];
              Lsum = ffma(ost[cc * PARTF + 65], wc, Lsum);
              O = ffma(ost[cc * PARTF + tl], wc, O);
            }
          }
          team_sync(team);
        }
        if (tl < 64) {
          const __half r = __float2half_rn(__fdiv_rn(O, Lsum));
          const __half r2 = __shfl_down_sync(0xffffffffu, r, 1);
          if ((tl & 1) == 0) ll_store(ws->attn_w + (h * HD + tl) / 2, pack2(r, r2), ep);
        }
      }
      STAMP();
      CSTAMP(3);

      if (n_out > 0) {
        ll_gather(ws->attn_w, HID, ep, sm.xs, err);
        __syncthreads();
        mbar_wait(&sm.bar[1], parC);
        gemv_stage<HID, false>(bufC, n_out, lb + BIAS_OUT, sm.xs, warp, lane, sm.stage16);
        __syncthreads();
        const bool withhold = a.fault && cta == a.fault - 1 && a.step_base + step >= 2;
        if (tid < (n_out >> 1) && !withhold)
          ll_store(ws->ya_w + ((row0_out + 2 * tid) >> 1), *reinterpret_cast<const uint32_t*>(sm.stage16 + 2 * tid), ep);
      } else {
        __syncthreads();
        mbar_wait(&sm.bar[1], parC);
      }
      parC ^= 1;
      if (tid == 0) {
        if (L + 1 < NL) refill(bufC, W.wo[L + 1], row0_out, n_out, HID, &sm.bar[1]);
        else refill(bufC, W.lm_head, row0_lm + a.rows_qkv, lmC, HID, &sm.bar[1]);
      }
      STAMP();
      CSTAMP(4);

      {
        float v[4];
        residual_in(ws->ya_w, ep, v);
        mbar_wait(&sm.lnbar[0], parL1);
        parL1 ^= 1;
        layernorm_1024(v, sm.ln1, sm.ln1 + HID, sm.red, tid);
        publish_x(v, true);
      }
      __syncthreads();
      if (tid == 0) fill_ln(sm.ln1, W.ln1g[(L + 1) % NL], W.ln1b[(L + 1) % NL], &sm.lnbar[0]);
      mbar_wait(&sm.bar[2], parA);
      parA ^= 1;
      gemv_stage<HID, true>(bufA, n_fc1, lb + BIAS_FC1, sm.xs, warp, lane, sm.stage16);
      __syncthreads();
      if (tid < (n_fc1 >> 1))
        ll_store(ws->f_w + ((row0_fc1 + 2 * tid) >> 1), *reinterpret_cast<const uint32_t*>(sm.stage16 + 2 * tid), ep);
      if (tid == 0) {
        if (L + 1 < NL) refill(bufA, W.w1[L + 1], row0_fc1, n_fc1, HID, &sm.bar[2]);
        else refill(bufA, W.lm_head, row0_lm + a.rows_qkv + a.rows_out, lmA, HID, &sm.bar[2]);
      }
      STAMP();
      CSTAMP(5);

      if (n_fc2 > 0) {
        ll_gather(ws->f_w, FFN, ep, sm.xs, err);
        __syncthreads();
        mbar_wait(&sm.bar[3], parB);
        gemv_stage<FFN, false>(bufB, n_fc2, lb + BIAS_FC2, sm.xs, warp, lane, sm.stage16);
        __syncthreads();
        if (tid < (n_fc2 >> 1))
          ll_store(ws->yb_w + ((row0_fc2 + 2 * tid) >> 1), *reinterpret_cast<const uint32_t*>(sm.stage16 + 2 * tid), ep);
      } else {
        __syncthreads();
        mbar_wait(&sm.bar[3], parB);
      }
      parB ^= 1;
      if (tid == 0) {
        refill(bufB, W.w2[(L + 1 < NL) ? L + 1 : 0], row0_fc2, n_fc2, FFN, &sm.bar[3]);
        fill_bias(sm.bias[bsel], ws->bias_cta + ((size_t)((L + 2) % NL) * 160 + cta) * 128, &sm.bbar[bsel]);
      }
      lc++;
      STAMP();
      CSTAMP(6);
    }

    const uint32_t epc = (uint32_t)(a.step_base + step) + 1u;
    {
      float v[4];
      residual_in(ws->yb_w, ep0 + (uint32_t)NL - 1u, v);
      mbar_wait(&sm.lnbar[1], parL2);
      parL2 ^= 1;
      layernorm_1024(v, sm.ln2, sm.ln2 + HID, sm.red, tid);
      publish_x(v, false);
    }
    __syncthreads();
    if (tid == 0) fill_ln(sm.ln2, W.ln2g[0], W.ln2b[0], &sm.lnbar[1]);
    mbar_wait(&sm.bar[0], parD);
    mbar_wait(&sm.bar[1], parC);
    mbar_wait(&sm.bar[2], parA);
    parD ^= 1; parC ^= 1; parA ^= 1;
    gemv_stage<HID, false>(bufD, n_lm, nullptr, sm.xs, warp, lane, sm.stage16);
    __syncthreads();
    float bestv = -INFINITY;
    int besti = 0x7fffffff;
    if (tid < n_lm) {
      const __half hv = sm.stage16[tid];
      if (a.logits_out) a.logits_out[(long)gen * W.vocab + row0_lm + tid] = hv;
      bestv = __half2float(hv);
      besti = row0_lm + tid;
    }
    if (warp < 2) {
#pragma unroll
      for (int o = 16; o > 0; o >>= 1) {
        const float ov = __shfl_xor_sync(0xffffffffu, bestv, o);
        const int oi = __shfl_xor_sync(0xffffffffu, besti, o);
        if (ov > bestv || (ov == bestv && oi < besti)) { bestv = ov; besti = oi; }
      }
      if (lane == 0) { sm.bval[warp] = bestv; sm.bidx[warp] = besti; }
    }
    __syncthreads();
    if (tid == 0) {
      float bv = sm.bval[0];
      int bi = sm.bidx[0];
      if (sm.bval[1] > bv || (sm.bval[1] == bv && sm.bidx[1] < bi)) { bv = sm.bval[1]; bi = sm.bidx[1]; }
      __threadfence();
      ll_store(ws->cand_w + 2 * cta, __float_as_uint(bv), epc);
      ll_store(ws->cand_w + 2 * cta + 1, (uint32_t)bi, epc);
      refill(bufD, W.wqkv[0], row0_qkv, n_qkv, HID, &sm.bar[0]);
      refill(bufC, W.wo[0], row0_out, n_out, HID, &sm.bar[1]);
      refill(bufA, W.w1[0], row0_fc1, n_fc1, HID, &sm.bar[2]);
    }
    {
      float bv = -INFINITY;
      int bi = 0x7fffffff;
      if (tid < ncta) {
        const uint2 d = ll_wait2(ws->cand_w + 2 * tid, epc, err);
        bv = __uint_as_float(d.x);
        bi = (int)d.y;
      }
#pragma unroll
      for (int o = 16; o > 0; o >>= 1) {
        const float ov = __shfl_xor_sync(0xffffffffu, bv, o);
        const int oi = __shfl_xor_sync(0xffffffffu, bi, o);
        if (ov > bv || (ov == bv && oi < bi)) { bv = ov; bi = oi; }
      }
      __syncthreads();
      if (lane == 0) { sm.bval[warp] = bv; sm.bidx[warp] = bi; }
      if (tid == 0) sm.errflag = *reinterpret_cast<volatile int*>(&ws->error);
      __syncthreads();
      bv = sm.bval[0];
      bi = sm.bidx[0];
      for (int w2 = 1; w2 < MG_WARPS; w2++)
        if (sm.bval[w2] > bv || (sm.bval[w2] == bv && sm.bidx[w2] < bi)) { bv = sm.bval[w2]; bi = sm.bidx[w2]; }
      if (sm.errflag) break;
      int ntok = bi;
      if (a.forced) ntok = a.forced[gen];
      if (fin) ntok = a.pad_id;
      if (cta == 0 && tid == 0) {
        if (gen < a.max_new) a.out_ids[gen] = ntok;
        if (!fin) a.s.lens[0] = gen + 1;
      }
      if (!fin && ntok == a.eos_id) fin = 1;
      tok = ntok;
      gen += 1;
      pos += 1;
      __syncthreads();
    }
    STAMP();
  }

  mbar_wait(&sm.bar[0], parD);
  mbar_wait(&sm.bar[1], parC);
  mbar_wait(&sm.bar[2], parA);
  mbar_wait(&sm.bar[3], parB);
  mbar_wait(&sm.lnbar[0], parL1);
  mbar_wait(&sm.lnbar[1], parL2);
  mbar_wait(&sm.bbar[0], parB0);
  mbar_wait(&sm.bbar[1], parB1);
  if (cta == 0 && tid == 0) {
    const int e = *reinterpret_cast<volatile int*>(&ws->error);
    a.s.pos[0] = pos; a.s.gen[0] = gen; a.s.tok[0] = tok; a.s.finished[0] = e ? 1 : fin;
    if (e) a.s.lens[0] = -1;
    if (a.nkeys_next) *a.nkeys_next = pos + 1;
    if (a.all_done) *a.all_done = e ? 1 : fin;
  }
}

static int g_mega_sms = 0;
size_t mega_workspace_bytes() { return sizeof(MegaWs) + 256; }

static int mega_sms() {
  if (!g_mega_sms) {
    int dev = 0;
    cudaGetDevice(&dev);
    cudaDeviceGetAttribute(&g_mega_sms, cudaDevAttrMultiProcessorCount, dev);
    if (g_mega_sms <= 0 || g_mega_sms > 160) g_mega_sms = 132;
  }
  return g_mega_sms;
}
static inline int mega_rpc(int N) { return (((N + mega_sms() - 1) / mega_sms()) + 1) & ~1; }

__global__ void mega_pack_bias_kernel(MegaWs* ws, int rq, int ro, int r1, int r2) {
  const int L = blockIdx.y, cta = blockIdx.x, t = threadIdx.x;
  const ma_decoder_weights& W = ws->w;
  __half v = __float2half_rn(0.0f);
  if (t < BIAS_OUT) {
    const int n = cta * rq + t;
    if (t < rq && n < QKV) v = reinterpret_cast<const __half*>(W.bqkv[L])[n];
  } else if (t < BIAS_FC1) {
    const int i = t - BIAS_OUT, n = cta * ro + i;
    if (i < ro && n < HID) v = reinterpret_cast<const __half*>(W.bo[L])[n];
  } else if (t < BIAS_FC2) {
    const int i = t - BIAS_FC1, n = cta * r1 + i;
    if (i < r1 && n < FFN) v = reinterpret_cast<const __half*>(W.b1[L])[n];
  } else {
    const int i = t - BIAS_FC2, n = cta * r2 + i;
    if (i < r2 && n < HID) v = reinterpret_cast<const __half*>(W.b2[L])[n];
  }
  ws->bias_cta[((size_t)L * 160 + cta) * 128 + t] = v;
}

int mega_prepare(const ma_decoder_weights* w, void* mega_ws, cudaStream_t st) {
  MegaWs* ws = reinterpret_cast<MegaWs*>(mega_ws);
  if (cudaMemsetAsync(ws, 0, offsetof(MegaWs, bias_cta), st) != cudaSuccess) return 1;
  if (cudaMemcpyAsync(&ws->w, w, sizeof(ma_decoder_weights), cudaMemcpyHostToDevice, st) != cudaSuccess) return 1;
  const int rq = mega_rpc(QKV), ro = mega_rpc(HID), r1 = mega_rpc(FFN), r2 = mega_rpc(HID);
  if (rq > 32 || ro > 16 || r1 > 64 || r2 > 16) {
    set_error("mega: rows per CTA out of range");
    return 1;
  }
  mega_pack_bias_kernel<<<dim3(160, w->n_layers), 128, 0, st>>>(ws, rq, ro, r1, r2);
  count_launch();
  return check_launch("mega_pack_bias_kernel") ? 0 : 1;
}

static int g_mega_fault = 0;
void mega_set_debug(unsigned long long timeout_ns, int fault) {
  if (timeout_ns) {
    const unsigned long long polls = timeout_ns / 400ull + 2048ull;
    const unsigned v = polls > 0xffffffffull ? 0xffffffffu : (unsigned)polls;
    cudaMemcpyToSymbol(c_spin_limit, &v, sizeof(v));
  }
  g_mega_fault = fault;
}
bool mega_fits(int tmax) { return tmax <= MAX_CHUNKS * MA_ATTN_CHUNK; }
int mega_supported() {
  static int ok = -1;
  if (ok < 0) {
    const int sms = mega_sms(), r1 = mega_rpc(FFN), ro = mega_rpc(HID);
    const int grid = (FFN + r1 - 1) / r1;
    ok = (grid <= sms && grid >= NHEAD && grid - NHEAD >= (HID + ro - 1) / ro && mega_rpc(QKV) <= 32 && ro <= 16 && r1 <= 64) ? 1 : 0;
    if (!ok) set_error("mega: unsupported SM count %d", sms);
  }
  return ok;
}
int mega_error_flag_offset() { return (int)offsetof(MegaWs, error); }
int mega_trace_offset() { return (int)offsetof(MegaWs, trace); }
int mega_trace_cta_offset() { return (int)offsetof(MegaWs, trace_cta); }

int mega_enqueue(const ma_decoder_weights* w, SeqState s, int tmax, __half* kv, void* mega_ws, const SampleArgs& sa,
                 int n_steps, int step_base, int trace, cudaStream_t st) {
  if (tmax > MAX_CHUNKS * MA_ATTN_CHUNK) {
    set_error("mega: tmax=%d exceeds %d keys", tmax, MAX_CHUNKS * MA_ATTN_CHUNK);
    return 1;
  }
  const int sms = mega_sms();
  auto rpc = [&](int N) { return mega_rpc(N); };
  MegaArgs a;
  memset(&a, 0, sizeof(a));
  a.ws = reinterpret_cast<MegaWs*>(mega_ws);
  a.s = s;
  a.kv = kv;
  a.T = tmax;
  a.n_steps = n_steps;
  a.step_base = step_base;
  a.max_new = sa.max_new; a.eos_id = sa.eos_id; a.pad_id = sa.pad_id;
  a.rows_qkv = rpc(QKV); a.rows_out = rpc(HID); a.rows_fc1 = rpc(FFN); a.rows_fc2 = rpc(HID); a.rows_lm = rpc(w->vocab);
  a.out_ids = sa.out_ids; a.forced = sa.forced; a.logits_out = sa.logits_out; a.all_done = sa.all_done;
  a.nkeys_next = sa.nkeys_next;
  a.trace = trace;
  a.fault = g_mega_fault;
  if (a.rows_lm > a.rows_qkv + a.rows_out + a.rows_fc1 || a.rows_lm > 64 || a.rows_fc1 > 64) {
    set_error("mega: rows per CTA out of range (lm %d, fc1 %d)", a.rows_lm, a.rows_fc1);
    return 1;
  }
  const int grid = (FFN + a.rows_fc1 - 1) / a.rows_fc1;
  if (grid > sms || (w->vocab + a.rows_lm - 1) / a.rows_lm != grid || grid < NHEAD) {
    set_error("mega: unsupported SM count %d (grid %d)", sms, grid);
    return 1;
  }
  if (grid - NHEAD < (HID + a.rows_out - 1) / a.rows_out) {
    set_error("mega: the last %d CTAs must not own out_proj rows (grid %d)", NHEAD, grid);
    return 1;
  }
  const size_t smem = sizeof(MegaSmem) + ((size_t)(a.rows_qkv + a.rows_out + a.rows_fc1) * HID + (size_t)a.rows_fc2 * FFN) * 2;
  static size_t attr_set = 0;
  if (smem > attr_set) {
    if (cudaFuncSetAttribute(decode_mega_kernel, cudaFuncAttributeMaxDynamicSharedMemorySize, (int)smem) != cudaSuccess) {
      set_error("mega: cannot get %zu bytes of shared memory", smem);
      cudaGetLastError();
      return 1;
    }
    attr_set = smem;
  }
  cudaLaunchConfig_t cfg = {};
  cfg.gridDim = dim3(grid);
  cfg.blockDim = dim3(MG_THREADS);
  cfg.dynamicSmemBytes = smem;
  cfg.stream = st;
  cudaLaunchAttribute at[1];
  at[0].id = cudaLaunchAttributeCooperative;
  at[0].val.cooperative = 1;
  cfg.attrs = at;
  cfg.numAttrs = 1;
  cudaLaunchKernelEx(&cfg, decode_mega_kernel, a);
  count_launch();
  return check_launch("decode_mega_kernel") ? 0 : 1;
}

}
```

meshanything_b200/csrc/internal.h:

```cpp
#pragma once
#include <cuda_fp16.h>
#include <cuda_runtime.h>
#include <stdint.h>

#include "../../include/meshanything_b200.h"

namespace ma {

constexpr int HID = 1024;
constexpr int NHEAD = 16;
constexpr int HD = 64;
constexpr int FFN = 4096;
constexpr int PREFIX = 257;
constexpr int QKV = 3 * HID;

struct SeqState {
  int* pos;
  int* gen;
  int* tok;
  int* finished;
  int* lens;
  int* sid;
};

void set_error(const char* fmt, ...);
void count_launch(int n = 1);
bool check_launch(const char* what);

int launch_linear(const __half* W, const __half* bias, const __half* x, int ldx, __half* y, int ldy, int M, int N,
                  int K, int epi, cudaStream_t st);

bool attention_tc_supported(int ldq, int ldo, long T, long Tpad, int nkeys, const void* q, const void* K, const void* Vt,
                            const void* out);
int launch_attention_tc(const __half* q, int ldq, const __half* K, const __half* Vt, long T, long Tpad, int H,
                        int rows_per_slot, int n_slots, int nkeys, float scale, __half* out, int ldo, cudaStream_t st);
int launch_scatter_heads_t(const __half* src, int ld, int col0, int head_stride, int H, int n, long Tpad, int n_slots,
                           __half* dst, cudaStream_t st);

bool linear_tc_supported(int M, int N, int K, int ldx, int ldy, const void* x, const void* W, const void* y);
int launch_linear_tc(const __half* W, const __half* bias, const __half* x, int ldx, __half* y, int ldy, int M, int N,
                     int K, int epi, cudaStream_t st);

size_t linear_ws_scratch_bytes();
void linear_ws_set_mode(int cluster);
int linear_ws_mode();
bool linear_ws_supported(int M, int N, int K, int ldx, const void* x, const void* W);
int launch_linear_ws(const __half* W, const __half* bias, const __half* x, int ldx, __half* y, int ldy, int M, int N,
                     int K, int epi, void* scratch, cudaStream_t st, bool pdl = false);

size_t attention_scratch_bytes(int M, int H, int max_keys);
int launch_attention_decode(const __half* qkv, int ldq, __half* K, __half* V, long T, const int* nkeys, int max_keys,
                            int M, float scale, __half* out, int ldo, void* scratch, bool pdl, cudaStream_t st);
int launch_attention(const __half* q, int ldq, const __half* K, const __half* V, long T, int H, int rows_per_slot,
                     const int* slots, const int* nkeys, int max_keys, int M, float scale, __half* out, int ldo,
                     void* scratch, cudaStream_t st);

int launch_layernorm(const float* x, const __half* res16, const float* gamma, const float* beta, float eps, int M,
                     int W, float* out32, __half* out16, cudaStream_t st, bool pdl = false);
int launch_embed_prefix(const ma_decoder_weights* w, const float* prefix, int B, float* hres, __half* x16, int* nkeys,
                        cudaStream_t st);
int launch_embed_tokens(const ma_decoder_weights* w, SeqState s, int B, float* hres, __half* x16, int* nkeys,
                        cudaStream_t st);
int launch_kv_append(const __half* qkv, int M, int rows_per_slot, const int* nkeys, __half* kc, __half* vc, long T,
                     cudaStream_t st);
int launch_gather_rows(const __half* src, int ld, int row0, int stride, int B, __half* dst, cudaStream_t st);
struct SampleArgs {
  const __half* logits;
  int vocab, B, max_new, eos_id, pad_id;
  int do_sample, top_k;
  float top_p;
  unsigned long long seed;
  SeqState s;
  int first;
  int32_t* out_ids;
  const int32_t* forced;
  __half* logits_out;
  int* all_done;
  int* nkeys_next;
  int32_t* support_out;
  int32_t* token_out;
  int row0, nrows;
  int slots;
};
int launch_sample(const SampleArgs& a, cudaStream_t st);
int launch_fill_i32(int32_t* p, int v, long n, cudaStream_t st);

int* fast_nkeys_ptr(void* fast_ws);
size_t fast_workspace_bytes();
int fast_step_enqueue(const ma_decoder_weights* w, SeqState s, int tmax, __half* kv, void* fast_ws,
                      const SampleArgs& sa, bool pdl, cudaStream_t st);


size_t mega_workspace_bytes();
int mega_prepare(const ma_decoder_weights* w, void* mega_ws, cudaStream_t st);
int mega_enqueue(const ma_decoder_weights* w, SeqState s, int tmax, __half* kv, void* mega_ws, const SampleArgs& sa,
                 int n_steps, int step_base, int trace, cudaStream_t st);
int mega_supported();
bool mega_fits(int tmax);
void mega_set_debug(unsigned long long timeout_ns, int fault);
int mega_error_flag_offset();
int mega_trace_offset();
int mega_trace_cta_offset();

}
```

Baseline: 1312.

## Balance persistent decoder row split across all SMs and restage LN/KV prefetch

Replaces the ceil-based rows-per-CTA split with an even pair-wise partition over min(SMs,160) CTAs, so every SM gets a near-equal share of qkv/out/fc1/fc2/lm rows and the grid always equals the SM count. The two layernorm shared buffers are merged into one, with the other LN parameters only prefetched to L2. KV register preloading before the layer is replaced by an L2 bulk prefetch of the current layer's chunks. This frees shared memory and evens out load, at the cost of losing the early KV register preload and serializing LN parameter fills.

```diff
diff --git a/include/meshanything_b200.h b/include/meshanything_b200.h
--- a/include/meshanything_b200.h
+++ b/include/meshanything_b200.h
@@ -96,6 +96,7 @@
 int ma_decoder_debug(void* ws, int B, int tmax, int what, void* host_out, int nbytes);
 void ma_mega_set_debug(unsigned long long timeout_ns, int fault);
 int ma_decode_persistent_supported(void);
+int ma_decode_persistent_plan(int sms, int smem_per_block, int vocab, int32_t* out);
 
 
 int ma_linear_tc_f16(const void* W, const void* bias, const void* x, int ldx, void* y, int ldy, int M, int N, int K,
diff --git a/meshanything_b200/capi.py b/meshanything_b200/capi.py
--- a/meshanything_b200/capi.py
+++ b/meshanything_b200/capi.py
@@ -40,6 +40,7 @@
     "ma_decode_slots_init", "ma_decode_slot_prefill", "ma_decode_slots_step", "ma_decode_slots_poll",
     "ma_mega_set_debug", "ma_linear_ws_set_mode", "ma_decode_slots_seek", "ma_decode_slot_stream", "ma_linear_ws_scratch_bytes", "ma_linear_ws_f16",
     "ma_sample_surface_workspace_bytes", "ma_sample_surface", "ma_tensor_core_linear_counts", "ma_decode_persistent_supported",
+    "ma_decode_persistent_plan",
 ]
 
 
@@ -94,6 +95,8 @@
     L.ma_mega_set_debug.restype = None
     L.ma_decode_persistent_supported.argtypes = []
     L.ma_decode_persistent_supported.restype = C.c_int
+    L.ma_decode_persistent_plan.argtypes = [C.c_int, C.c_int, C.c_int, _vp]
+    L.ma_decode_persistent_plan.restype = C.c_int
     L.ma_encoder_workspace_bytes.argtypes = [C.c_int]
     L.ma_encoder_workspace_bytes.restype = C.c_size_t
     L.ma_encoder_forward.argtypes = [_vp, _vp, C.c_int, _vp, _vp, _vp, _vp]
diff --git a/meshanything_b200/csrc/api.cu b/meshanything_b200/csrc/api.cu
--- a/meshanything_b200/csrc/api.cu
+++ b/meshanything_b200/csrc/api.cu
@@ -596,6 +596,9 @@
 
 void ma_mega_set_debug(unsigned long long timeout_ns, int fault) { mega_set_debug(timeout_ns, fault); }
 int ma_decode_persistent_supported(void) { return mega_supported(); }
+int ma_decode_persistent_plan(int sms, int smem_per_block, int vocab, int32_t* out) {
+  return mega_plan_query(sms, smem_per_block, vocab, out);
+}
 
 int ma_decoder_debug(void* ws_, int B, int tmax, int what, void* host_out, int nbytes) {
   DecWs ws = carve(ws_, B, tmax, 8195 + 61);
diff --git a/meshanything_b200/csrc/decode_mega.cu b/meshanything_b200/csrc/decode_mega.cu
--- a/meshanything_b200/csrc/decode_mega.cu
+++ b/meshanything_b200/csrc/decode_mega.cu
@@ -1,3 +1,5 @@
+#include <cstdio>
+
 #include "canon.cuh"
 #include "internal.h"
 
@@ -8,6 +10,7 @@
 constexpr int TEAM = 256;
 constexpr int PARTF = 66;
 constexpr int MAX_CHUNKS = 72;
+constexpr int MAX_GRID = 160;
 
 struct MegaWs {
   uint2 qkv_w[QKV / 2];
@@ -19,13 +22,20 @@
   int error;
   int pad_[3];
   unsigned long long trace[1280];
-  unsigned long long trace_cta[160 * 8];
+  unsigned long long trace_cta[MAX_GRID * 8];
   ma_decoder_weights w;
   alignas(256) uint2 part_w[NHEAD * MAX_CHUNKS * PARTF];
-  alignas(256) __half bias_cta[MA_MAX_LAYERS * 160 * 128];
+  alignas(256) __half bias_cta[MA_MAX_LAYERS * MAX_GRID * 128];
 };
 
 constexpr int BIAS_QKV = 0, BIAS_OUT = 32, BIAS_FC1 = 48, BIAS_FC2 = 112;
+
+__host__ __device__ __forceinline__ int mega_row0(int N, int c, int G) {
+  const long long pairs = (N + 1) >> 1;
+  const int r = 2 * (int)(((long long)c * pairs) / G);
+  return r < N ? r : N;
+}
+__host__ __device__ __forceinline__ int mega_rows_max(int N, int G) { return 2 * ((((N + 1) >> 1) + G - 1) / G); }
 
 struct MegaArgs {
   MegaWs* ws;
@@ -33,7 +43,7 @@
   __half* kv;
   long T;
   int n_steps, step_base, max_new, eos_id, pad_id;
-  int rows_qkv, rows_out, rows_fc1, rows_fc2, rows_lm;
+  int rows_qkv, rows_out, rows_fc1, rows_fc2;
   int32_t* out_ids;
   const int32_t* forced;
   __half* logits_out;
@@ -135,13 +145,13 @@
 
 struct alignas(128) MegaSmem {
   uint64_t bar[4];
-  uint64_t lnbar[2];
+  uint64_t lnbar;
   uint64_t bbar[2];
-  alignas(16) float ln1[2 * HID];
-  alignas(16) float ln2[2 * HID];
+  alignas(16) float ln[2 * HID];
   alignas(16) __half bias[2][128];
   ma_decoder_weights wtab;
   int errflag;
+  int blk[11];
   float red[2][8];
   float wmax[2][8];
   float ared[2][8][65];
@@ -275,6 +285,10 @@
   bulk_g2s(dst, g, HID * 4, bar);
   bulk_g2s(dst + HID, b, HID * 4, bar);
 }
+__device__ __forceinline__ void prefetch_ln(const float* g, const float* b) {
+  asm volatile("cp.async.bulk.prefetch.L2.global [%0], %1;" ::"l"(g), "r"(HID * 4) : "memory");
+  asm volatile("cp.async.bulk.prefetch.L2.global [%0], %1;" ::"l"(b), "r"(HID * 4) : "memory");
+}
 __device__ __forceinline__ void fill_bias(__half* dst, const __half* src, uint64_t* bar) {
   fence_proxy_async();
   mbar_expect_tx(bar, 256);
@@ -306,24 +320,33 @@
   int* err = &ws->error;
 
   const int cta = blockIdx.x, ncta = gridDim.x;
-  const int row0_qkv = cta * a.rows_qkv, n_qkv = max(0, min(a.rows_qkv, QKV - row0_qkv));
-  const int row0_out = cta * a.rows_out, n_out = max(0, min(a.rows_out, HID - row0_out));
-  const int row0_fc1 = cta * a.rows_fc1, n_fc1 = max(0, min(a.rows_fc1, FFN - row0_fc1));
-  const int row0_fc2 = cta * a.rows_fc2, n_fc2 = max(0, min(a.rows_fc2, HID - row0_fc2));
-  const int row0_lm = cta * a.rows_lm, n_lm = max(0, min(a.rows_lm, W.vocab - row0_lm));
-  const int lmD = min(n_lm, a.rows_qkv), lmC = max(0, min(n_lm, a.rows_qkv + a.rows_out) - a.rows_qkv),
-            lmA = max(0, n_lm - a.rows_qkv - a.rows_out);
-
-  uint32_t parD = 0, parC = 0, parA = 0, parB = 0, parL1 = 0, parL2 = 0, parB0 = 0, parB1 = 0;
+  const int &row0_qkv = sm.blk[0], &n_qkv = sm.blk[1], &row0_out = sm.blk[2], &n_out = sm.blk[3];
+  const int &row0_fc1 = sm.blk[4], &n_fc1 = sm.blk[5], &row0_lm = sm.blk[6], &n_lm = sm.blk[7];
+  const int &lmD = sm.blk[8], &lmC = sm.blk[9], &lmA = sm.blk[10];
+  const int &row0_fc2 = row0_out, &n_fc2 = n_out;
+  if (tid == 0) {
+    int* b = sm.blk;
+    const int Ns[4] = {QKV, HID, FFN, W.vocab};
+    for (int i = 0; i < 4; i++) {
+      b[2 * i] = mega_row0(Ns[i], cta, ncta);
+      b[2 * i + 1] = mega_row0(Ns[i], cta + 1, ncta) - b[2 * i];
+    }
+    b[8] = min(b[7], a.rows_qkv);
+    b[9] = max(0, min(b[7], a.rows_qkv + a.rows_out) - a.rows_qkv);
+    b[10] = max(0, b[7] - a.rows_qkv - a.rows_out);
+  }
+
+  uint32_t parD = 0, parC = 0, parA = 0, parB = 0, parL = 0, parB0 = 0, parB1 = 0;
   int lc = 0;
   if (tid == 0) {
     for (int i = 0; i < 4; i++) mbar_init(&sm.bar[i], 1);
-    for (int i = 0; i < 2; i++) { mbar_init(&sm.lnbar[i], 1); mbar_init(&sm.bbar[i], 1); }
+    mbar_init(&sm.lnbar, 1);
+    for (int i = 0; i < 2; i++) mbar_init(&sm.bbar[i], 1);
     mbar_fence_init();
-    fill_ln(sm.ln1, W.ln1g[0], W.ln1b[0], &sm.lnbar[0]);
-    fill_ln(sm.ln2, W.ln2g[0], W.ln2b[0], &sm.lnbar[1]);
-    fill_bias(sm.bias[0], ws->bias_cta + ((size_t)0 * 160 + cta) * 128, &sm.bbar[0]);
-    fill_bias(sm.bias[1], ws->bias_cta + ((size_t)(NL > 1 ? 1 : 0) * 160 + cta) * 128, &sm.bbar[1]);
+    fill_ln(sm.ln, W.ln1g[0], W.ln1b[0], &sm.lnbar);
+    prefetch_ln(W.ln2g[0], W.ln2b[0]);
+    fill_bias(sm.bias[0], ws->bias_cta + ((size_t)0 * MAX_GRID + cta) * 128, &sm.bbar[0]);
+    fill_bias(sm.bias[1], ws->bias_cta + ((size_t)(NL > 1 ? 1 : 0) * MAX_GRID + cta) * 128, &sm.bbar[1]);
     refill(bufD, W.wqkv[0], row0_qkv, n_qkv, HID, &sm.bar[0]);
     refill(bufC, W.wo[0], row0_out, n_out, HID, &sm.bar[1]);
     refill(bufA, W.w1[0], row0_fc1, n_fc1, HID, &sm.bar[2]);
@@ -335,7 +358,7 @@
   unsigned long long* tr = (a.trace && cta == 0 && tid == 0) ? ws->trace : nullptr;
   int tri = 0;
 #define STAMP() do { if (tr && tri < 1270) tr[tri++] = gtimer(); } while (0)
-#define CSTAMP(k) do { if (a.trace && tid == 0 && step == 1 && L == NL / 2) ws->trace_cta[cta * 8 + (k)] = gtimer(); } while (0)
+#define CSTAMP(k) do { if (a.trace && tid == 0 && L == NL / 2) ws->trace_cta[cta * 8 + (k)] = gtimer(); } while (0)
 
   auto publish_x = [&](const float* v, bool keep_hres) {
     if (tid < 256) {
@@ -365,6 +388,7 @@
     const int nch = (nkeys + MA_ATTN_CHUNK - 1) / MA_ATTN_CHUNK;
     const int nitems = nch * NHEAD;
     const uint32_t ep0 = (uint32_t)(a.step_base + step) * (uint32_t)NL + 1u;
+    tri = 0;
     STAMP();
 
     for (int L = 0; L < NL; L++) {
@@ -374,21 +398,15 @@
       __half* kc = a.kv + ((size_t)(L * 2 + 0)) * NHEAD * T * HD;
       __half* vc = a.kv + ((size_t)(L * 2 + 1)) * NHEAD * T * HD;
 
-      uint4 kreg[8], vreg[8];
-      int item = team * ncta + (ncta - 1 - cta);
-      if (item < nitems) {
-        const int c = item >> 4, h = item & 15;
-        const long base = ((long)h * T + (long)c * MA_ATTN_CHUNK) * HD;
-#pragma unroll
-        for (int rho = 0; rho < 8; rho++) {
-          const int r = 32 * rho + 4 * wt + grp;
-          if (c * MA_ATTN_CHUNK + r < pos) {
-            kreg[rho] = ldcg16(kc + base + (long)r * HD + 8 * li);
-            vreg[rho] = ldcg16(vc + base + (long)r * HD + 8 * li);
-          }
-        }
-      }
-
+      if (tl == 0) {
+        for (int it2 = team * ncta + (ncta - 1 - cta); it2 < nitems; it2 += 2 * ncta) {
+          const int c2 = it2 >> 4, h2 = it2 & 15;
+          const uint32_t bytes = (uint32_t)min(MA_ATTN_CHUNK, nkeys - c2 * MA_ATTN_CHUNK) * HD * 2;
+          const long off = ((long)h2 * T + (long)c2 * MA_ATTN_CHUNK) * HD;
+          asm volatile("cp.async.bulk.prefetch.L2.global [%0], %1;" ::"l"(kc + off), "r"(bytes) : "memory");
+          asm volatile("cp.async.bulk.prefetch.L2.global [%0], %1;" ::"l"(vc + off), "r"(bytes) : "memory");
+        }
+      }
       {
         float v[4] = {0.0f, 0.0f, 0.0f, 0.0f};
         if (L == 0) {
@@ -418,14 +436,17 @@
           }
         } else {
           residual_in(ws->yb_w, ep - 1, v);
-          mbar_wait(&sm.lnbar[1], parL2);
-          parL2 ^= 1;
-          layernorm_1024(v, sm.ln2, sm.ln2 + HID, sm.red, tid);
+          mbar_wait(&sm.lnbar, parL);
+          parL ^= 1;
+          layernorm_1024(v, sm.ln, sm.ln + HID, sm.red, tid);
         }
         publish_x(v, true);
       }
       __syncthreads();
-      if (L > 0 && tid == 0) fill_ln(sm.ln2, W.ln2g[L], W.ln2b[L], &sm.lnbar[1]);
+      if (L > 0 && tid == 0) {
+        fill_ln(sm.ln, W.ln1g[L], W.ln1b[L], &sm.lnbar);
+        prefetch_ln(W.ln2g[L], W.ln2b[L]);
+      }
       STAMP();
       CSTAMP(0);
       mbar_wait(&sm.bbar[bsel], bsel ? parB1 : parB0);
@@ -454,7 +475,8 @@
       STAMP();
       CSTAMP(1);
 
-      for (int it = 0; item < nitems; item += 2 * ncta, it++) {
+      uint4 kreg[8], vreg[8];
+      for (int item = team * ncta + (ncta - 1 - cta); item < nitems; item += 2 * ncta) {
         const int c = item >> 4, h = item & 15;
         const int len = min(MA_ATTN_CHUNK, nkeys - c * MA_ATTN_CHUNK);
         const long base = ((long)h * T + (long)c * MA_ATTN_CHUNK) * HD;
@@ -462,7 +484,7 @@
 #pragma unroll
         for (int rho = 0; rho < 8; rho++) {
           const int r = 32 * rho + 4 * wt + grp;
-          if (r < len && it > 0 && r != cur) {
+          if (r < len && r != cur) {
             kreg[rho] = ldcg16(kc + base + (long)r * HD + 8 * li);
             vreg[rho] = ldcg16(vc + base + (long)r * HD + 8 * li);
           }
@@ -513,6 +535,7 @@
         float lmax = own_valid ? s_own : -INFINITY;
         lmax = warp_max(lmax);
         team_sync(team);
+        CSTAMP(7);
         if (lane == 0) sm.wmax[team][wt] = lmax;
         team_sync(team);
         float cmax = sm.wmax[team][0];
@@ -556,18 +579,6 @@
           uint2* part = ws->part_w + ((long)h * MAX_CHUNKS + c) * PARTF;
           ll_store(part + (tl < 64 ? tl : 65), __float_as_uint(rsum), ep);
           if (tl == 64) ll_store(part + 64, __float_as_uint(cmax), ep);
-        }
-      }
-      if (tl == 0) {
-        const int Ln = (L + 1 < NL) ? L + 1 : 0;
-        const __half* kn = a.kv + ((size_t)(Ln * 2 + 0)) * NHEAD * T * HD;
-        const __half* vn = a.kv + ((size_t)(Ln * 2 + 1)) * NHEAD * T * HD;
-        for (int it2 = team * ncta + (ncta - 1 - cta); it2 < nitems; it2 += 2 * ncta) {
-          const int c2 = it2 >> 4, h2 = it2 & 15;
-          const uint32_t bytes = (uint32_t)min(MA_ATTN_CHUNK, nkeys - c2 * MA_ATTN_CHUNK) * HD * 2;
-          const long off = ((long)h2 * T + (long)c2 * MA_ATTN_CHUNK) * HD;
-          asm volatile("cp.async.bulk.prefetch.L2.global [%0], %1;" ::"l"(kn + off), "r"(bytes) : "memory");
-          asm volatile("cp.async.bulk.prefetch.L2.global [%0], %1;" ::"l"(vn + off), "r"(bytes) : "memory");
         }
       }
       STAMP();
@@ -666,13 +677,16 @@
       {
         float v[4];
         residual_in(ws->ya_w, ep, v);
-        mbar_wait(&sm.lnbar[0], parL1);
-        parL1 ^= 1;
-        layernorm_1024(v, sm.ln1, sm.ln1 + HID, sm.red, tid);
+        mbar_wait(&sm.lnbar, parL);
+        parL ^= 1;
+        layernorm_1024(v, sm.ln, sm.ln + HID, sm.red, tid);
         publish_x(v, true);
       }
       __syncthreads();
-      if (tid == 0) fill_ln(sm.ln1, W.ln1g[(L + 1) % NL], W.ln1b[(L + 1) % NL], &sm.lnbar[0]);
+      if (tid == 0) {
+        fill_ln(sm.ln, W.ln2g[L], W.ln2b[L], &sm.lnbar);
+        prefetch_ln(W.ln1g[(L + 1) % NL], W.ln1b[(L + 1) % NL]);
+      }
       mbar_wait(&sm.bar[2], parA);
       parA ^= 1;
       gemv_stage<HID, true>(bufA, n_fc1, lb + BIAS_FC1, sm.xs, warp, lane, sm.stage16);
@@ -701,7 +715,7 @@
       parB ^= 1;
       if (tid == 0) {
         refill(bufB, W.w2[(L + 1 < NL) ? L + 1 : 0], row0_fc2, n_fc2, FFN, &sm.bar[3]);
-        fill_bias(sm.bias[bsel], ws->bias_cta + ((size_t)((L + 2) % NL) * 160 + cta) * 128, &sm.bbar[bsel]);
+        fill_bias(sm.bias[bsel], ws->bias_cta + ((size_t)((L + 2) % NL) * MAX_GRID + cta) * 128, &sm.bbar[bsel]);
       }
       lc++;
       STAMP();
@@ -712,13 +726,16 @@
     {
       float v[4];
       residual_in(ws->yb_w, ep0 + (uint32_t)NL - 1u, v);
-      mbar_wait(&sm.lnbar[1], parL2);
-      parL2 ^= 1;
-      layernorm_1024(v, sm.ln2, sm.ln2 + HID, sm.red, tid);
+      mbar_wait(&sm.lnbar, parL);
+      parL ^= 1;
+      layernorm_1024(v, sm.ln, sm.ln + HID, sm.red, tid);
       publish_x(v, false);
     }
     __syncthreads();
-    if (tid == 0) fill_ln(sm.ln2, W.ln2g[0], W.ln2b[0], &sm.lnbar[1]);
+    if (tid == 0) {
+      fill_ln(sm.ln, W.ln1g[0], W.ln1b[0], &sm.lnbar);
+      prefetch_ln(W.ln2g[0], W.ln2b[0]);
+    }
     mbar_wait(&sm.bar[0], parD);
     mbar_wait(&sm.bar[1], parC);
     mbar_wait(&sm.bar[2], parA);
@@ -797,8 +814,7 @@
   mbar_wait(&sm.bar[1], parC);
   mbar_wait(&sm.bar[2], parA);
   mbar_wait(&sm.bar[3], parB);
-  mbar_wait(&sm.lnbar[0], parL1);
-  mbar_wait(&sm.lnbar[1], parL2);
+  mbar_wait(&sm.lnbar, parL);
   mbar_wait(&sm.bbar[0], parB0);
   mbar_wait(&sm.bbar[1], parB1);
   if (cta == 0 && tid == 0) {
@@ -810,50 +826,83 @@
   }
 }
 
-static int g_mega_sms = 0;
 size_t mega_workspace_bytes() { return sizeof(MegaWs) + 256; }
 
-static int mega_sms() {
-  if (!g_mega_sms) {
+constexpr int MEGA_VOCAB = 8195;
+
+struct MegaPlan {
+  int grid;
+  int rows_qkv, rows_out, rows_fc1, rows_fc2, rows_lm;
+  size_t smem;
+};
+static bool mega_plan(int sms, long smem_optin, int vocab, MegaPlan& p, char* why, size_t nwhy) {
+  p = MegaPlan{};
+  p.grid = sms < MAX_GRID ? sms : MAX_GRID;
+  if (p.grid < NHEAD) {
+    snprintf(why, nwhy, "%d SMs: the kernel needs at least %d", sms, NHEAD);
+    return false;
+  }
+  p.rows_qkv = mega_rows_max(QKV, p.grid);
+  p.rows_out = mega_rows_max(HID, p.grid);
+  p.rows_fc1 = mega_rows_max(FFN, p.grid);
+  p.rows_fc2 = mega_rows_max(HID, p.grid);
+  p.rows_lm = mega_rows_max(vocab, p.grid);
+  p.smem = sizeof(MegaSmem) + ((size_t)(p.rows_qkv + p.rows_out + p.rows_fc1) * HID + (size_t)p.rows_fc2 * FFN) * 2;
+  if (FFN / 2 < p.grid) {
+    snprintf(why, nwhy, "%d CTAs: not every CTA owns fc1 rows", p.grid);
+    return false;
+  }
+  if (p.rows_qkv > BIAS_OUT - BIAS_QKV || p.rows_out > BIAS_FC1 - BIAS_OUT || p.rows_fc1 > BIAS_FC2 - BIAS_FC1 ||
+      p.rows_fc2 > 128 - BIAS_FC2 || p.rows_lm > 64 || p.rows_lm > p.rows_qkv + p.rows_out + p.rows_fc1) {
+    snprintf(why, nwhy, "%d SMs: rows per CTA out of range (qkv %d, out_proj %d, fc1 %d, fc2 %d, lm_head %d)", sms,
+             p.rows_qkv, p.rows_out, p.rows_fc1, p.rows_fc2, p.rows_lm);
+    return false;
+  }
+  if ((long)p.smem > smem_optin) {
+    snprintf(why, nwhy, "%d SMs: a CTA needs %zu bytes of shared memory, the device allows %ld", sms, p.smem, smem_optin);
+    return false;
+  }
+  return true;
+}
+static bool mega_device_plan(int vocab, MegaPlan& p) {
+  static int sms = -1, optin = 0;
+  if (sms < 0) {
     int dev = 0;
-    cudaGetDevice(&dev);
-    cudaDeviceGetAttribute(&g_mega_sms, cudaDevAttrMultiProcessorCount, dev);
-    if (g_mega_sms <= 0 || g_mega_sms > 160) g_mega_sms = 132;
-  }
-  return g_mega_sms;
-}
-static inline int mega_rpc(int N) { return (((N + mega_sms() - 1) / mega_sms()) + 1) & ~1; }
-
-__global__ void mega_pack_bias_kernel(MegaWs* ws, int rq, int ro, int r1, int r2) {
+    if (cudaGetDevice(&dev) != cudaSuccess || cudaDeviceGetAttribute(&sms, cudaDevAttrMultiProcessorCount, dev) != cudaSuccess ||
+        cudaDeviceGetAttribute(&optin, cudaDevAttrMaxSharedMemoryPerBlockOptin, dev) != cudaSuccess) {
+      sms = 0;
+      optin = 0;
+      cudaGetLastError();
+    }
+  }
+  char why[200];
+  if (sms > 0 && mega_plan(sms, optin, vocab, p, why, sizeof(why))) return true;
+  set_error("mega: %s", sms > 0 ? why : "no CUDA device");
+  return false;
+}
+
+__global__ void mega_pack_bias_kernel(MegaWs* ws, int grid) {
   const int L = blockIdx.y, cta = blockIdx.x, t = threadIdx.x;
   const ma_decoder_weights& W = ws->w;
-  __half v = __float2half_rn(0.0f);
-  if (t < BIAS_OUT) {
-    const int n = cta * rq + t;
-    if (t < rq && n < QKV) v = reinterpret_cast<const __half*>(W.bqkv[L])[n];
-  } else if (t < BIAS_FC1) {
-    const int i = t - BIAS_OUT, n = cta * ro + i;
-    if (i < ro && n < HID) v = reinterpret_cast<const __half*>(W.bo[L])[n];
-  } else if (t < BIAS_FC2) {
-    const int i = t - BIAS_FC1, n = cta * r1 + i;
-    if (i < r1 && n < FFN) v = reinterpret_cast<const __half*>(W.b1[L])[n];
-  } else {
-    const int i = t - BIAS_FC2, n = cta * r2 + i;
-    if (i < r2 && n < HID) v = reinterpret_cast<const __half*>(W.b2[L])[n];
-  }
-  ws->bias_cta[((size_t)L * 160 + cta) * 128 + t] = v;
+  auto pick = [&](const void* b, int N, int i) {
+    const int n = mega_row0(N, cta, grid) + i;
+    return n < mega_row0(N, cta + 1, grid) ? reinterpret_cast<const __half*>(b)[n] : __float2half_rn(0.0f);
+  };
+  __half v;
+  if (t < BIAS_OUT) v = pick(W.bqkv[L], QKV, t - BIAS_QKV);
+  else if (t < BIAS_FC1) v = pick(W.bo[L], HID, t - BIAS_OUT);
+  else if (t < BIAS_FC2) v = pick(W.b1[L], FFN, t - BIAS_FC1);
+  else v = pick(W.b2[L], HID, t - BIAS_FC2);
+  ws->bias_cta[((size_t)L * MAX_GRID + cta) * 128 + t] = v;
 }
 
 int mega_prepare(const ma_decoder_weights* w, void* mega_ws, cudaStream_t st) {
   MegaWs* ws = reinterpret_cast<MegaWs*>(mega_ws);
+  MegaPlan p;
+  if (!mega_device_plan(w->vocab, p)) return 1;
   if (cudaMemsetAsync(ws, 0, offsetof(MegaWs, bias_cta), st) != cudaSuccess) return 1;
   if (cudaMemcpyAsync(&ws->w, w, sizeof(ma_decoder_weights), cudaMemcpyHostToDevice, st) != cudaSuccess) return 1;
-  const int rq = mega_rpc(QKV), ro = mega_rpc(HID), r1 = mega_rpc(FFN), r2 = mega_rpc(HID);
-  if (rq > 32 || ro > 16 || r1 > 64 || r2 > 16) {
-    set_error("mega: rows per CTA out of range");
-    return 1;
-  }
-  mega_pack_bias_kernel<<<dim3(160, w->n_layers), 128, 0, st>>>(ws, rq, ro, r1, r2);
+  mega_pack_bias_kernel<<<dim3(p.grid, w->n_layers), 128, 0, st>>>(ws, p.grid);
   count_launch();
   return check_launch("mega_pack_bias_kernel") ? 0 : 1;
 }
@@ -870,13 +919,25 @@
 bool mega_fits(int tmax) { return tmax <= MAX_CHUNKS * MA_ATTN_CHUNK; }
 int mega_supported() {
   static int ok = -1;
+  static char why[512] = "";
   if (ok < 0) {
-    const int sms = mega_sms(), r1 = mega_rpc(FFN), ro = mega_rpc(HID);
-    const int grid = (FFN + r1 - 1) / r1;
-    ok = (grid <= sms && grid >= NHEAD && grid - NHEAD >= (HID + ro - 1) / ro && mega_rpc(QKV) <= 32 && ro <= 16 && r1 <= 64) ? 1 : 0;
-    if (!ok) set_error("mega: unsupported SM count %d", sms);
-  }
+    MegaPlan p;
+    ok = mega_device_plan(MEGA_VOCAB, p) ? 1 : 0;
+    if (!ok) snprintf(why, sizeof(why), "%s", ma_last_error());
+  }
+  if (!ok) set_error("%s", why);
   return ok;
+}
+int mega_plan_query(int sms, long smem_optin, int vocab, int* out) {
+  MegaPlan p;
+  char why[200];
+  const bool ok = mega_plan(sms, smem_optin, vocab, p, why, sizeof(why));
+  if (out) {
+    out[0] = p.grid; out[1] = p.rows_qkv; out[2] = p.rows_out; out[3] = p.rows_fc1; out[4] = p.rows_fc2;
+    out[5] = p.rows_lm; out[6] = (int)p.smem;
+  }
+  if (!ok) set_error("mega: %s", why);
+  return ok ? 1 : 0;
 }
 int mega_error_flag_offset() { return (int)offsetof(MegaWs, error); }
 int mega_trace_offset() { return (int)offsetof(MegaWs, trace); }
@@ -888,8 +949,8 @@
     set_error("mega: tmax=%d exceeds %d keys", tmax, MAX_CHUNKS * MA_ATTN_CHUNK);
     return 1;
   }
-  const int sms = mega_sms();
-  auto rpc = [&](int N) { return mega_rpc(N); };
+  MegaPlan p;
+  if (!mega_device_plan(w->vocab, p)) return 1;
   MegaArgs a;
   memset(&a, 0, sizeof(a));
   a.ws = reinterpret_cast<MegaWs*>(mega_ws);
@@ -899,25 +960,12 @@
   a.n_steps = n_steps;
   a.step_base = step_base;
   a.max_new = sa.max_new; a.eos_id = sa.eos_id; a.pad_id = sa.pad_id;
-  a.rows_qkv = rpc(QKV); a.rows_out = rpc(HID); a.rows_fc1 = rpc(FFN); a.rows_fc2 = rpc(HID); a.rows_lm = rpc(w->vocab);
+  a.rows_qkv = p.rows_qkv; a.rows_out = p.rows_out; a.rows_fc1 = p.rows_fc1; a.rows_fc2 = p.rows_fc2;
   a.out_ids = sa.out_ids; a.forced = sa.forced; a.logits_out = sa.logits_out; a.all_done = sa.all_done;
   a.nkeys_next = sa.nkeys_next;
   a.trace = trace;
   a.fault = g_mega_fault;
-  if (a.rows_lm > a.rows_qkv + a.rows_out + a.rows_fc1 || a.rows_lm > 64 || a.rows_fc1 > 64) {
-    set_error("mega: rows per CTA out of range (lm %d, fc1 %d)", a.rows_lm, a.rows_fc1);
-    return 1;
-  }
-  const int grid = (FFN + a.rows_fc1 - 1) / a.rows_fc1;
-  if (grid > sms || (w->vocab + a.rows_lm - 1) / a.rows_lm != grid || grid < NHEAD) {
-    set_error("mega: unsupported SM count %d (grid %d)", sms, grid);
-    return 1;
-  }
-  if (grid - NHEAD < (HID + a.rows_out - 1) / a.rows_out) {
-    set_error("mega: the last %d CTAs must not own out_proj rows (grid %d)", NHEAD, grid);
-    return 1;
-  }
-  const size_t smem = sizeof(MegaSmem) + ((size_t)(a.rows_qkv + a.rows_out + a.rows_fc1) * HID + (size_t)a.rows_fc2 * FFN) * 2;
+  const size_t smem = p.smem;
   static size_t attr_set = 0;
   if (smem > attr_set) {
     if (cudaFuncSetAttribute(decode_mega_kernel, cudaFuncAttributeMaxDynamicSharedMemorySize, (int)smem) != cudaSuccess) {
@@ -928,7 +976,7 @@
     attr_set = smem;
   }
   cudaLaunchConfig_t cfg = {};
-  cfg.gridDim = dim3(grid);
+  cfg.gridDim = dim3(p.grid);
   cfg.blockDim = dim3(MG_THREADS);
   cfg.dynamicSmemBytes = smem;
   cfg.stream = st;
diff --git a/meshanything_b200/csrc/internal.h b/meshanything_b200/csrc/internal.h
--- a/meshanything_b200/csrc/internal.h
+++ b/meshanything_b200/csrc/internal.h
@@ -96,6 +96,7 @@
 int mega_enqueue(const ma_decoder_weights* w, SeqState s, int tmax, __half* kv, void* mega_ws, const SampleArgs& sa,
                  int n_steps, int step_base, int trace, cudaStream_t st);
 int mega_supported();
+int mega_plan_query(int sms, long smem_optin, int vocab, int* out);
 bool mega_fits(int tmax);
 void mega_set_debug(unsigned long long timeout_ns, int fault);
 int mega_error_flag_offset();
```

New measurement: 1331, median of 6. 1.4% higher.
